# Zhen-Dong/HAWQ

Measured on NVIDIA H100. Metric: images/sec ResNet-50 W8A8 & W4A4 @batch128, 1/2/4/8xH100; % int-TC roofline, higher is better.
Workload: dtype int8

## Files before the change

hawq_b200/csrc/api.cu:

```cuda
#include <cmath>
#include <cstdarg>
#include <cstdio>
#include <cstring>

#include <cstdlib>

#include "conv_igemm.cuh"
#include "elementwise.cuh"
#include "stem.cuh"

using namespace hawq;

struct hawq_handle {
  int device;
  int sm_count;
  int32_t* status;
};

static thread_local char g_err[512] = "";
static long long g_kernel_count[8] = {0, 0, 0, 0, 0, 0, 0, 0};

static int fail(int code, const char* fmt, ...) {
  va_list ap;
  va_start(ap, fmt);
  vsnprintf(g_err, sizeof(g_err), fmt, ap);
  va_end(ap);
  return code;
}

#define CUDA_TRY(expr)                                                                         \
  do {                                                                                         \
    cudaError_t _e = (expr);                                                                   \
    if (_e != cudaSuccess) return fail(HAWQ_ERR_CUDA, "%s: %s", #expr, cudaGetErrorString(_e)); \
  } while (0)

static int launch_check(const char* what) {
  cudaError_t e = cudaGetLastError();
  if (e != cudaSuccess) return fail(HAWQ_ERR_CUDA, "%s launch: %s", what, cudaGetErrorString(e));
  return HAWQ_OK;
}

static int grid_for(long long work_items, int sm_count) {
  long long blocks = (work_items + 255) / 256;
  const long long cap = (long long)sm_count * 16;
  if (blocks > cap) blocks = cap;
  if (blocks < 1) blocks = 1;
  return (int)blocks;
}

template <int BN, bool A4, int FAM, bool DUAL>
static int set_conv_attr1() {
  CUDA_TRY(cudaFuncSetAttribute(conv_igemm_kernel<BN, A4, FAM, DUAL>, cudaFuncAttributeMaxDynamicSharedMemorySize,
                                ConvSmem<BN, A4, DUAL>::TOTAL));
  CUDA_TRY(cudaFuncSetAttribute(conv_igemm_kernel<BN, A4, FAM, DUAL>, cudaFuncAttributePreferredSharedMemoryCarveout,
                                cudaSharedmemCarveoutMaxShared));
  return HAWQ_OK;
}
template <int BN, bool A4>
static int set_conv_attr() {
  int rc;
  if ((rc = set_conv_attr1<BN, A4, FAM_REQUANT, false>()) || (rc = set_conv_attr1<BN, A4, FAM_RESIDUAL, false>()) ||
      (rc = set_conv_attr1<BN, A4, FAM_STORE, false>()))
    return rc;
  return HAWQ_OK;
}

static dim3 conv_grid(long long M, int Cout, int BN) { return dim3((unsigned)((M + CONV_BM - 1) / CONV_BM * (Cout / BN)), 1, 1); }

template <int BN, bool A4>
static void launch_conv(const ConvParams& p, cudaStream_t s) {
  const int smem = ConvSmem<BN, A4, false>::TOTAL;
  const dim3 grid = conv_grid(p.M, p.Cout, BN);
  if (p.mode == HAWQ_EPI_REQUANT) conv_igemm_kernel<BN, A4, FAM_REQUANT, false><<<grid, CONV_THREADS, smem, s>>>(p);
  else if (p.mode == HAWQ_EPI_RESIDUAL) conv_igemm_kernel<BN, A4, FAM_RESIDUAL, false><<<grid, CONV_THREADS, smem, s>>>(p);
  else conv_igemm_kernel<BN, A4, FAM_STORE, false><<<grid, CONV_THREADS, smem, s>>>(p);
}
template <bool A4>
static void launch_conv_dual(const ConvParams& p, cudaStream_t s) {
  conv_igemm_kernel<64, A4, FAM_RESIDUAL, true><<<conv_grid(p.M, p.Cout, 64), CONV_THREADS, ConvSmem<64, A4, true>::TOTAL, s>>>(p);
}

extern "C" {

int hawq_abi_version(void) { return HAWQ_ABI_VERSION; }
const char* hawq_last_error(void) { return g_err; }

int hawq_create(int device, hawq_handle** out) {
  if (!out) return fail(HAWQ_ERR_BAD_ARG, "hawq_create: out is null");
  CUDA_TRY(cudaSetDevice(device));
  cudaDeviceProp prop;
  CUDA_TRY(cudaGetDeviceProperties(&prop, device));
  if (prop.major != 9 || prop.minor != 0)
    return fail(HAWQ_ERR_UNSUPPORTED, "hawq_create: device sm_%d%d is not Hopper sm_90 (the library is built for sm_90a)", prop.major, prop.minor);
  hawq_handle* h = new hawq_handle();
  h->device = device;
  h->sm_count = prop.multiProcessorCount;
  h->status = nullptr;
  CUDA_TRY(cudaMalloc(&h->status, sizeof(int32_t)));
  CUDA_TRY(cudaMemset(h->status, 0, sizeof(int32_t)));
  int rc;
  CUDA_TRY(cudaFuncSetAttribute(linear_dp4a_kernel, cudaFuncAttributeMaxDynamicSharedMemorySize, linear_smem_bytes(LIN_MAX_K)));
  if ((rc = set_conv_attr<128, false>()) || (rc = set_conv_attr<64, false>()) || (rc = set_conv_attr<128, true>()) ||
      (rc = set_conv_attr<64, true>()) || (rc = set_conv_attr1<64, false, FAM_RESIDUAL, true>()) ||
      (rc = set_conv_attr1<64, true, FAM_RESIDUAL, true>()))
    return rc;
  *out = h;
  return HAWQ_OK;
}

int hawq_destroy(hawq_handle* h) {
  if (!h) return HAWQ_OK;
  cudaFree(h->status);
  delete h;
  return HAWQ_OK;
}

int hawq_sm_count(const hawq_handle* h) { return h ? h->sm_count : 0; }

int hawq_reset_status(hawq_handle* h, void* stream) {
  if (!h) return fail(HAWQ_ERR_BAD_ARG, "null handle");
  CUDA_TRY(cudaMemsetAsync(h->status, 0, sizeof(int32_t), (cudaStream_t)stream));
  return HAWQ_OK;
}

int hawq_get_status(hawq_handle* h, void* stream, int32_t* host_flags) {
  if (!h || !host_flags) return fail(HAWQ_ERR_BAD_ARG, "null argument");
  CUDA_TRY(cudaMemcpyAsync(host_flags, h->status, sizeof(int32_t), cudaMemcpyDeviceToHost, (cudaStream_t)stream));
  CUDA_TRY(cudaStreamSynchronize((cudaStream_t)stream));
  return HAWQ_OK;
}

int hawq_copy_status(hawq_handle* h, int32_t* dst, void* stream) {
  if (!h || !dst) return fail(HAWQ_ERR_BAD_ARG, "null argument");
  CUDA_TRY(cudaMemcpyAsync(dst, h->status, sizeof(int32_t), cudaMemcpyDeviceToDevice, (cudaStream_t)stream));
  return HAWQ_OK;
}

static void set_bias_window(ConvParams& p, int a_bits) {
  long long bound = (long long)p.K * (a_bits == 4 ? 15 * 128 : 128 * 128);
  if (bound > 2147483648ll) bound = 2147483648ll;
  p.bias_lo = (int)(bound - 2147483648ll);
  p.bias_hi = (int)(2147483647ll - bound);
}

static int check_me(uint32_t m, int e, const char* what) {
  if (e < 1 || e > 62 || m > 0x80000000u) return fail(HAWQ_ERR_BAD_ARG, "%s: dyadic pair out of range (m=%u e=%d)", what, m, e);
  return HAWQ_OK;
}

int hawq_conv2d(hawq_handle* h, const hawq_conv_desc* d, const hawq_epilogue_desc* ep, const void* x, const int8_t* w,
                const hawq_chan* chan, const void* res, const hawq_chan* res_chan, const float* fscale, void* out,
                void* out_low, void* stream) {
  if (!h || !d || !ep || !x || !w || !chan) return fail(HAWQ_ERR_BAD_ARG, "hawq_conv2d: null argument");
  if (d->N < 1 || d->H < 1 || d->W < 1 || d->kh < 1 || d->kw < 1 || d->stride < 1 || d->pad < 0)
    return fail(HAWQ_ERR_BAD_ARG, "hawq_conv2d: bad geometry");
  if (d->a_bits != 8 && d->a_bits != 4) return fail(HAWQ_ERR_UNSUPPORTED, "hawq_conv2d: a_bits must be 4 or 8");
  if (d->Cin % 64 != 0 || d->Cout % 64 != 0)
    return fail(HAWQ_ERR_UNSUPPORTED, "hawq_conv2d: Cin (%d) and Cout (%d) must be multiples of 64", d->Cin, d->Cout);
  const int Ho = (d->H + 2 * d->pad - d->kh) / d->stride + 1;
  const int Wo = (d->W + 2 * d->pad - d->kw) / d->stride + 1;
  if (Ho < 1 || Wo < 1) return fail(HAWQ_ERR_BAD_ARG, "hawq_conv2d: empty output");
  const long long M = (long long)d->N * Ho * Wo;
  if (M > 0x7fffff00ll || (long long)d->N * d->H * d->W > 0x7fffff00ll) return fail(HAWQ_ERR_UNSUPPORTED, "hawq_conv2d: too many pixels");

  ConvParams p;
  memset(&p, 0, sizeof(p));
  p.x = (const uint8_t*)x; p.w = w; p.chan = chan; p.res = res; p.res_chan = res_chan; p.fscale = fscale;
  p.out = out; p.out_low = out_low; p.status = h->status;
  p.N = d->N; p.H = d->H; p.W = d->W; p.Cin = d->Cin; p.Cout = d->Cout; p.KH = d->kh; p.KW = d->kw;
  p.stride = d->stride; p.pad = d->pad; p.Ho = Ho; p.Wo = Wo; p.M = (int)M; p.K = d->kh * d->kw * d->Cin;
  p.cin_chunks = d->Cin / 64;
  p.x_pix_bytes = d->Cin * d->a_bits / 8;
  p.mode = ep->mode; p.relu = ep->relu; p.out_bits = ep->out_bits; p.lo = ep->clamp_lo; p.hi = ep->clamp_hi;
  p.res_kind = ep->res_kind; p.res_bits = ep->res_bits; p.res_m = ep->res_m; p.res_e = ep->res_e;
  p.y_bits = ep->y_bits; p.low_bits = ep->low_bits; p.low_m = ep->low_m; p.low_e = ep->low_e;
  p.low_lo = ep->low_lo; p.low_hi = ep->low_hi; p.cout_store = ep->cout_store;
  set_bias_window(p, d->a_bits);
  p.check_ovf = ep->mode == HAWQ_EPI_RESIDUAL && (ep->flags & (HAWQ_EP_RATIOS_LE_ONE | HAWQ_EP_RATIOS_LE_2P20)) != 0;
  if (ep->mode == HAWQ_EPI_RESIDUAL) {
    const bool low_over_one = ep->low_bits != 0 && !dyadic_is_fast(ep->low_m, ep->low_e);
    p.scalar_over_one = (ep->res_kind == 0 && !dyadic_is_fast(ep->res_m, ep->res_e)) || low_over_one;
    p.scalar_unchecked = (ep->res_kind == 0 && !dyadic_is_wide(ep->res_m, ep->res_e)) || low_over_one;
  }

  switch (ep->mode) {
    case HAWQ_EPI_REQUANT:
      if (!out) return fail(HAWQ_ERR_BAD_ARG, "hawq_conv2d: REQUANT needs out");
      if (ep->out_bits != 4 && ep->out_bits != 8 && ep->out_bits != 16 && ep->out_bits != 32)
        return fail(HAWQ_ERR_BAD_ARG, "hawq_conv2d: out_bits must be 4/8/16/32");
      if (ep->clamp_lo > ep->clamp_hi) return fail(HAWQ_ERR_BAD_ARG, "hawq_conv2d: empty clamp range");
      break;
    case HAWQ_EPI_RESIDUAL:
      if (!res) return fail(HAWQ_ERR_BAD_ARG, "hawq_conv2d: RESIDUAL needs res");
      if (ep->res_kind == 1) {
        if (!res_chan) return fail(HAWQ_ERR_BAD_ARG, "hawq_conv2d: res_kind 1 needs res_chan");
      } else if (ep->res_kind == 0) {
        if (ep->res_bits != 16 && ep->res_bits != 32) return fail(HAWQ_ERR_BAD_ARG, "hawq_conv2d: res_bits must be 16/32");
        int rc = check_me(ep->res_m, ep->res_e, "hawq_conv2d residual");
        if (rc) return rc;
      } else return fail(HAWQ_ERR_BAD_ARG, "hawq_conv2d: res_kind must be 0/1");
      if (ep->y_bits != 0 && ep->y_bits != 16 && ep->y_bits != 32) return fail(HAWQ_ERR_BAD_ARG, "hawq_conv2d: y_bits must be 0/16/32");
      if (ep->y_bits == 16 && !ep->relu) return fail(HAWQ_ERR_BAD_ARG, "hawq_conv2d: uint16 residual stream requires relu");
      if (ep->y_bits && !out) return fail(HAWQ_ERR_BAD_ARG, "hawq_conv2d: y_bits set but out is null");
      if (ep->low_bits != 0 && ep->low_bits != 4 && ep->low_bits != 8) return fail(HAWQ_ERR_BAD_ARG, "hawq_conv2d: low_bits must be 0/4/8");
      if (ep->low_bits) {
        if (!out_low) return fail(HAWQ_ERR_BAD_ARG, "hawq_conv2d: low_bits set but out_low is null");
        int rc = check_me(ep->low_m, ep->low_e, "hawq_conv2d low-bit copy");
        if (rc) return rc;
      }
      if (!ep->y_bits && !ep->low_bits) return fail(HAWQ_ERR_BAD_ARG, "hawq_conv2d: RESIDUAL with no output");
      break;
    case HAWQ_EPI_RAW_I32:
      if (!out) return fail(HAWQ_ERR_BAD_ARG, "hawq_conv2d: RAW_I32 needs out");
      break;
    case HAWQ_EPI_DEQUANT_F32:
      if (!out || !fscale) return fail(HAWQ_ERR_BAD_ARG, "hawq_conv2d: DEQUANT_F32 needs out and fscale");
      if (ep->cout_store < 1 || ep->cout_store > d->Cout) return fail(HAWQ_ERR_BAD_ARG, "hawq_conv2d: bad cout_store");
      break;
    default:
      return fail(HAWQ_ERR_BAD_ARG, "hawq_conv2d: unknown epilogue mode %d", ep->mode);
  }

  const bool bn128 = (d->Cout % 128 == 0);
  if ((M + CONV_BM - 1) / CONV_BM * (d->Cout / (bn128 ? 128 : 64)) > 0x7fffffffll)
    return fail(HAWQ_ERR_UNSUPPORTED, "hawq_conv2d: more than 2^31 - 1 output tiles");
  ++g_kernel_count[0];
  cudaStream_t s = (cudaStream_t)stream;
  if (d->a_bits == 8) {
    if (bn128) launch_conv<128, false>(p, s);
    else launch_conv<64, false>(p, s);
  } else {
    if (bn128) launch_conv<128, true>(p, s);
    else launch_conv<64, true>(p, s);
  }
  return launch_check("conv_igemm");
}

int hawq_conv2d_dual(hawq_handle* h, const hawq_conv_desc* d, const hawq_epilogue_desc* ep, const void* x, const int8_t* w,
                     const hawq_chan* chan, const hawq_conv_desc* d2, const void* x2, const int8_t* w2, const hawq_chan* chan2,
                     void* out, void* out_low, void* stream) {
  if (!h || !d || !ep || !x || !w || !chan || !d2 || !x2 || !w2 || !chan2 || !out) return fail(HAWQ_ERR_BAD_ARG, "hawq_conv2d_dual: null argument");
  if (d->kh != 1 || d->kw != 1 || d->stride != 1 || d->pad != 0 || d2->kh != 1 || d2->kw != 1 || d2->pad != 0 || d2->stride < 1)
    return fail(HAWQ_ERR_UNSUPPORTED, "hawq_conv2d_dual: both convolutions must be 1x1 without padding (main stride 1)");
  if (d->N < 1 || d->H < 1 || d->W < 1 || d2->H < 1 || d2->W < 1) return fail(HAWQ_ERR_BAD_ARG, "hawq_conv2d_dual: bad geometry");
  if ((d->a_bits != 8 && d->a_bits != 4) || d2->a_bits != d->a_bits) return fail(HAWQ_ERR_UNSUPPORTED, "hawq_conv2d_dual: a_bits must be equal and 4 or 8");
  if (d->Cin % 64 || d2->Cin % 64 || d->Cout % 64 || d2->Cout != d->Cout) return fail(HAWQ_ERR_UNSUPPORTED, "hawq_conv2d_dual: channel counts must be multiples of 64 and Cout equal");
  if (d2->N != d->N || (d2->H - 1) / d2->stride + 1 != d->H || (d2->W - 1) / d2->stride + 1 != d->W)
    return fail(HAWQ_ERR_BAD_ARG, "hawq_conv2d_dual: the two convolutions have different output grids");
  if (d->w_layout != 1 || d2->w_layout != 1) return fail(HAWQ_ERR_UNSUPPORTED, "hawq_conv2d_dual: weights must carry the re-tiled copy (w_layout 1)");
  if (ep->mode != HAWQ_EPI_RESIDUAL || !ep->relu || ep->y_bits != 16) return fail(HAWQ_ERR_UNSUPPORTED, "hawq_conv2d_dual: RESIDUAL + relu + uint16 stream only");
  if (ep->low_bits != 0 && ep->low_bits != 4 && ep->low_bits != 8) return fail(HAWQ_ERR_BAD_ARG, "hawq_conv2d_dual: low_bits must be 0/4/8");
  if (ep->low_bits) {
    if (!out_low) return fail(HAWQ_ERR_BAD_ARG, "hawq_conv2d_dual: low_bits set but out_low is null");
    int rc = check_me(ep->low_m, ep->low_e, "hawq_conv2d_dual low-bit copy");
    if (rc) return rc;
    if (!dyadic_is_fast(ep->low_m, ep->low_e)) return fail(HAWQ_ERR_UNSUPPORTED, "hawq_conv2d_dual: low-bit ratio outside the fast range");
  }
  const bool ratios_one = (ep->flags & HAWQ_EP_RATIOS_LE_ONE) != 0;
  const bool ratios_wide = !ratios_one && (ep->flags & HAWQ_EP_RATIOS_LE_2P20) != 0;
  if (!ratios_one && !ratios_wide) return fail(HAWQ_ERR_UNSUPPORTED, "hawq_conv2d_dual: needs a ratio-range promise (flags)");
  const long long M = (long long)d->N * d->H * d->W;
  if (M > 0x7fffff00ll || (long long)d2->N * d2->H * d2->W > 0x7fffff00ll) return fail(HAWQ_ERR_UNSUPPORTED, "hawq_conv2d_dual: too many pixels");
  if ((M + CONV_BM - 1) / CONV_BM * (d->Cout / 64) > 0x7fffffffll)
    return fail(HAWQ_ERR_UNSUPPORTED, "hawq_conv2d_dual: more than 2^31 - 1 output tiles");

  ++g_kernel_count[4];
  ConvParams p;
  memset(&p, 0, sizeof(p));
  p.x = (const uint8_t*)x; p.w = w; p.chan = chan; p.res_chan = chan2; p.out = out; p.out_low = out_low; p.status = h->status;
  p.N = d->N; p.H = d->H; p.W = d->W; p.Cin = d->Cin; p.Cout = d->Cout; p.KH = 1; p.KW = 1; p.stride = 1; p.pad = 0;
  p.Ho = d->H; p.Wo = d->W; p.M = (int)M; p.K = d->Cin; p.cin_chunks = d->Cin / 64; p.x_pix_bytes = d->Cin * d->a_bits / 8;
  p.mode = HAWQ_EPI_RESIDUAL; p.relu = 1; p.res_kind = 1; p.res_bits = 32; p.y_bits = 16; p.low_bits = ep->low_bits; p.low_m = ep->low_m;
  p.low_e = ep->low_e; p.low_lo = ep->low_lo; p.low_hi = ep->low_hi;
  p.check_ovf = 1;
  set_bias_window(p, d->a_bits);
  p.x2 = (const uint8_t*)x2; p.w2 = w2; p.H2 = d2->H; p.W2 = d2->W; p.stride2 = d2->stride; p.cin_chunks2 = d2->Cin / 64;
  p.x2_pix_bytes = d2->Cin * d2->a_bits / 8;

  cudaStream_t s = (cudaStream_t)stream;
  if (d->a_bits == 8) launch_conv_dual<false>(p, s);
  else launch_conv_dual<true>(p, s);
  return launch_check("conv_dual");
}

int hawq_conv2d_i8(hawq_handle* h, const hawq_conv_desc* d, const hawq_epilogue_desc* ep, const void* x,
                   const int8_t* w, const hawq_chan* chan, const void* res, const hawq_chan* res_chan,
                   const float* fscale, void* out, void* out_low, void* stream) {
  if (d && d->a_bits != 8) return fail(HAWQ_ERR_BAD_ARG, "hawq_conv2d_i8: a_bits must be 8");
  return hawq_conv2d(h, d, ep, x, w, chan, res, res_chan, fscale, out, out_low, stream);
}

int hawq_conv2d_i4(hawq_handle* h, const hawq_conv_desc* d, const hawq_epilogue_desc* ep, const void* x,
                   const int8_t* w, const hawq_chan* chan, const void* res, const hawq_chan* res_chan,
                   const float* fscale, void* out, void* out_low, void* stream) {
  if (d && d->a_bits != 4) return fail(HAWQ_ERR_BAD_ARG, "hawq_conv2d_i4: a_bits must be 4");
  return hawq_conv2d(h, d, ep, x, w, chan, res, res_chan, fscale, out, out_low, stream);
}

int hawq_linear_i8(hawq_handle* h, int32_t N, int32_t K, int32_t Cout, int32_t Cout_pad, const int8_t* x,
                   const int8_t* w, const hawq_chan* chan, const float* fscale, float* out, void* stream) {
  if (Cout < 1 || Cout > Cout_pad) return fail(HAWQ_ERR_BAD_ARG, "hawq_linear_i8: bad Cout/Cout_pad");
  if (!h || !x || !w || !chan || !fscale || !out || N < 1 || K < 1) return fail(HAWQ_ERR_BAD_ARG, "hawq_linear_i8: null argument or empty shape");
  static const bool dp4a_enabled = [] { const char* e = getenv("HAWQ_B200_LINEAR_DP4A"); return !(e && e[0] == '0'); }();
  if (dp4a_enabled && K % LIN_SLAB == 0 && K <= LIN_MAX_K && Cout_pad % LIN_CH == 0 && N <= 65535 * LIN_ROWS) {
    const dim3 grid((unsigned)(Cout_pad / LIN_CH), (unsigned)((N + LIN_ROWS - 1) / LIN_ROWS), 1);
    linear_dp4a_kernel<<<grid, 256, linear_smem_bytes(K), (cudaStream_t)stream>>>(x, w, chan, fscale, out, N, K, Cout);
    return launch_check("linear_dp4a");
  }
  hawq_conv_desc d;
  memset(&d, 0, sizeof(d));
  d.N = N; d.H = 1; d.W = 1; d.Cin = K; d.Cout = Cout_pad; d.kh = 1; d.kw = 1; d.stride = 1; d.pad = 0; d.a_bits = 8;
  hawq_epilogue_desc ep;
  memset(&ep, 0, sizeof(ep));
  ep.mode = HAWQ_EPI_DEQUANT_F32;
  ep.cout_store = Cout;
  return hawq_conv2d(h, &d, &ep, x, w, chan, nullptr, nullptr, fscale, out, nullptr, stream);
}

int hawq_stem_conv_i8(hawq_handle* h, int32_t N, int32_t H, int32_t W, const int8_t* x, const int8_t* w,
                      const hawq_chan* chan, int32_t clamp_lo, int32_t clamp_hi, int16_t* out, void* stream) {
  if (!h || !x || !w || !chan || !out) return fail(HAWQ_ERR_BAD_ARG, "hawq_stem_conv_i8: null argument");
  if (N < 1 || H < 7 || W < 7) return fail(HAWQ_ERR_BAD_ARG, "hawq_stem_conv_i8: bad geometry");
  if (clamp_lo < -32768 || clamp_hi > 32767 || clamp_lo > clamp_hi) return fail(HAWQ_ERR_BAD_ARG, "hawq_stem_conv_i8: clamp must fit int16");
  if (N > 65535) return fail(HAWQ_ERR_UNSUPPORTED, "hawq_stem_conv_i8: N > 65535");
  const int Ho = (H + 6 - 7) / 2 + 1, Wo = (W + 6 - 7) / 2 + 1;
  const dim3 grid((Wo + STEM_TW - 1) / STEM_TW, (Ho + STEM_TH - 1) / STEM_TH, N);
  const long long tiles = (long long)N * grid.x * grid.y;
  const int ctas = (int)(tiles < 4LL * h->sm_count ? tiles : 4LL * h->sm_count);
  stem_conv_kernel<<<ctas, 256, 0, (cudaStream_t)stream>>>(x, (const uint32_t*)w, chan, N, H, W, Ho, Wo, clamp_lo, clamp_hi, out);
  return launch_check("stem_conv");
}

int hawq_stem_pool_i8(hawq_handle* h, int32_t N, int32_t H, int32_t W, const int8_t* x, const int8_t* w256, const hawq_chan* chan,
                      int32_t clamp_lo, int32_t clamp_hi, int32_t y_bits, void* y, int32_t low_bits, uint32_t low_m, int32_t low_e,
                      int32_t low_lo, int32_t low_hi, void* out_low, void* stream) {
  if (!h || !x || !w256 || !chan || !y) return fail(HAWQ_ERR_BAD_ARG, "hawq_stem_pool_i8: null argument");
  if (N < 1 || H < 7 || W < 7) return fail(HAWQ_ERR_BAD_ARG, "hawq_stem_pool_i8: bad geometry");
  if (clamp_lo < -32768 || clamp_hi > 32767 || clamp_lo > clamp_hi) return fail(HAWQ_ERR_BAD_ARG, "hawq_stem_pool_i8: clamp must fit int16");
  if ((y_bits != 16 && y_bits != 32) || (low_bits != 0 && low_bits != 4 && low_bits != 8) || (low_bits && !out_low))
    return fail(HAWQ_ERR_BAD_ARG, "hawq_stem_pool_i8: bad output description");
  if (low_bits) { int rc = check_me(low_m, low_e, "hawq_stem_pool_i8"); if (rc) return rc; }
  if (W % 16 != 0 || W > 256 || (low_bits && !dyadic_is_fast(low_m, low_e)))
    return fail(HAWQ_ERR_UNSUPPORTED, "hawq_stem_pool_i8: shape / ratio outside the fused kernel (use hawq_stem_conv_i8 + hawq_maxpool_requant)");
  if (N > 65535) return fail(HAWQ_ERR_UNSUPPORTED, "hawq_stem_pool_i8: N > 65535");
  const int Ho = (H + 6 - 7) / 2 + 1, Wo = (W + 6 - 7) / 2 + 1;
  const int Po = (Ho + 2 - 3) / 2 + 1, Qo = (Wo + 2 - 3) / 2 + 1;
  const long long tiles = (long long)N * ((Po + STEMP_PH - 1) / STEMP_PH) * ((Qo + STEMP_PW - 1) / STEMP_PW);
  const int ctas = (int)(tiles < 4LL * h->sm_count ? tiles : 4LL * h->sm_count);
  ++g_kernel_count[6];
  stem_pool_kernel<<<ctas, 256, 0, (cudaStream_t)stream>>>(x, (const uint32_t*)w256, chan, N, H, W, Ho, Wo, Po, Qo, clamp_lo, clamp_hi, y_bits, y,
                                                          low_bits, low_m, low_e, low_lo, low_hi, out_low);
  return launch_check("stem_pool");
}

int hawq_maxpool_requant(hawq_handle* h, int32_t N, int32_t H, int32_t W, int32_t C, const int16_t* x, int32_t y_bits,
                         void* y, int32_t low_bits, uint32_t low_m, int32_t low_e, int32_t low_lo, int32_t low_hi,
                         void* out_low, void* stream) {
  if (!h || !x) return fail(HAWQ_ERR_BAD_ARG, "hawq_maxpool_requant: null argument");
  if (C % 8 != 0) return fail(HAWQ_ERR_UNSUPPORTED, "hawq_maxpool_requant: C %% 8 != 0");
  if ((y_bits != 0 && y_bits != 16 && y_bits != 32) || (y_bits && !y)) return fail(HAWQ_ERR_BAD_ARG, "hawq_maxpool_requant: bad y");
  if ((low_bits != 0 && low_bits != 4 && low_bits != 8) || (low_bits && !out_low)) return fail(HAWQ_ERR_BAD_ARG, "hawq_maxpool_requant: bad low");
  if (low_bits) { int rc = check_me(low_m, low_e, "hawq_maxpool_requant"); if (rc) return rc; }
  const int Ho = (H + 2 - 3) / 2 + 1, Wo = (W + 2 - 3) / 2 + 1;
  const long long total = (long long)N * Ho * Wo * (C / 8);
  maxpool_requant_kernel<<<grid_for(total, h->sm_count), 256, 0, (cudaStream_t)stream>>>(
      x, N, H, W, C, Ho, Wo, y_bits, y, low_bits, low_m, low_e, low_lo, low_hi, out_low);
  return launch_check("maxpool_requant");
}

int hawq_avgpool_requant(hawq_handle* h, int32_t N, int32_t HW, int32_t C, int32_t x_bits, const void* x, uint32_t m,
                         int32_t e, int32_t lo, int32_t hi, int8_t* out, void* stream) {
  if (!h || !x || !out) return fail(HAWQ_ERR_BAD_ARG, "hawq_avgpool_requant: null argument");
  if (x_bits != 16 && x_bits != 32) return fail(HAWQ_ERR_BAD_ARG, "hawq_avgpool_requant: x_bits must be 16/32");
  if (lo < -128 || hi > 127) return fail(HAWQ_ERR_BAD_ARG, "hawq_avgpool_requant: clamp must fit int8");
  int rc = check_me(m, e, "hawq_avgpool_requant");
  if (rc) return rc;
  avgpool_requant_kernel<<<grid_for((long long)N * C, h->sm_count), 256, 0, (cudaStream_t)stream>>>(x, N, HW, C, x_bits, m, e, lo, hi, out);
  return launch_check("avgpool_requant");
}

int hawq_quantize_input_f32(hawq_handle* h, int32_t N, int32_t C, int32_t H, int32_t W, const float* x, float scale,
                            int32_t lo, int32_t hi, int8_t* out, void* stream) {
  if (!h || !x || !out) return fail(HAWQ_ERR_BAD_ARG, "hawq_quantize_input_f32: null argument");
  if (!(scale > 0.f)) return fail(HAWQ_ERR_BAD_ARG, "hawq_quantize_input_f32: scale must be > 0");
  if (lo < -128 || hi > 127) return fail(HAWQ_ERR_BAD_ARG, "hawq_quantize_input_f32: clamp must fit int8");
  const float inv = 1.0f / scale;
  quantize_input_kernel<<<grid_for((long long)N * H * W, h->sm_count), 256, 0, (cudaStream_t)stream>>>(x, N, C, H, W, inv, lo, hi, out);
  return launch_check("quantize_input");
}

int hawq_quantize_input_u8(hawq_handle* h, int32_t N, int32_t H, int32_t W, const uint8_t* x, const float* mean3,
                           const float* std3, float scale, int32_t lo, int32_t hi, int8_t* out, void* stream) {
  if (!h || !x || !out || !mean3 || !std3) return fail(HAWQ_ERR_BAD_ARG, "hawq_quantize_input_u8: null argument");
  if (N < 1 || H < 1 || W < 1) return fail(HAWQ_ERR_BAD_ARG, "hawq_quantize_input_u8: empty shape");
  if (!(scale > 0.f)) return fail(HAWQ_ERR_BAD_ARG, "hawq_quantize_input_u8: scale must be > 0");
  if (lo < -128 || hi > 127 || lo > hi) return fail(HAWQ_ERR_BAD_ARG, "hawq_quantize_input_u8: clamp must fit int8");
  for (int c = 0; c < 3; ++c)
    if (!(std3[c] > 0.f)) return fail(HAWQ_ERR_BAD_ARG, "hawq_quantize_input_u8: std must be > 0");
  const float inv = 1.0f / scale;
  const long long n_bytes = (long long)N * H * W * 3;
  quantize_input_u8_kernel<<<grid_for(n_bytes / 4 + 1, h->sm_count), 256, 0, (cudaStream_t)stream>>>(
      x, n_bytes, 3, mean3[0], mean3[1], mean3[2], std3[0], std3[1], std3[2], inv, lo, hi, out);
  return launch_check("quantize_input_u8");
}

int hawq_requant(hawq_handle* h, int64_t rows, int32_t C, int32_t x_bits, const void* x, const hawq_chan* chan,
                 int32_t chan_stride, int32_t relu, int32_t out_bits, int32_t lo, int32_t hi, void* out, void* stream) {
  if (!h || !x || !chan || !out) return fail(HAWQ_ERR_BAD_ARG, "hawq_requant: null argument");
  if (C % 8 != 0) return fail(HAWQ_ERR_UNSUPPORTED, "hawq_requant: C %% 8 != 0");
  if (x_bits != 16 && x_bits != 32) return fail(HAWQ_ERR_BAD_ARG, "hawq_requant: x_bits must be 16/32");
  if (out_bits != 4 && out_bits != 8 && out_bits != 16 && out_bits != 32) return fail(HAWQ_ERR_BAD_ARG, "hawq_requant: out_bits must be 4/8/16/32");
  if (chan_stride != 0 && chan_stride != 1) return fail(HAWQ_ERR_BAD_ARG, "hawq_requant: chan_stride must be 0/1");
  requant_kernel<<<grid_for(rows * (C / 8), h->sm_count), 256, 0, (cudaStream_t)stream>>>(x, rows, C, x_bits, chan, chan_stride, relu, out_bits, lo, hi, out);
  return launch_check("requant");
}

int hawq_add_requant(hawq_handle* h, int64_t rows, int32_t C, const int32_t* acc, const hawq_chan* chan,
                     const hawq_epilogue_desc* ep, const void* res, const hawq_chan* res_chan, void* y, void* out_low,
                     void* stream) {
  if (!h || !acc || !chan || !ep || !res) return fail(HAWQ_ERR_BAD_ARG, "hawq_add_requant: null argument");
  if (C % 8 != 0) return fail(HAWQ_ERR_UNSUPPORTED, "hawq_add_requant: C %% 8 != 0");
  if (ep->res_kind == 1 && !res_chan) return fail(HAWQ_ERR_BAD_ARG, "hawq_add_requant: res_kind 1 needs res_chan");
  if (ep->res_kind == 0) { int rc = check_me(ep->res_m, ep->res_e, "hawq_add_requant"); if (rc) return rc; }
  if (ep->y_bits == 16 && !ep->relu) return fail(HAWQ_ERR_BAD_ARG, "hawq_add_requant: uint16 residual stream requires relu");
  if ((ep->y_bits && !y) || (ep->low_bits && !out_low)) return fail(HAWQ_ERR_BAD_ARG, "hawq_add_requant: missing output");
  AddRequantParams p;
  p.acc = acc; p.chan = chan; p.res = res; p.res_chan = res_chan; p.y = y; p.out_low = out_low; p.status = h->status;
  p.rows = rows; p.C = C; p.relu = ep->relu; p.res_kind = ep->res_kind; p.res_bits = ep->res_bits; p.res_m = ep->res_m;
  p.res_e = ep->res_e; p.y_bits = ep->y_bits; p.low_bits = ep->low_bits; p.low_m = ep->low_m; p.low_e = ep->low_e;
  p.low_lo = ep->low_lo; p.low_hi = ep->low_hi;
  add_requant_kernel<<<grid_for(rows * (C / 8), h->sm_count), 256, 0, (cudaStream_t)stream>>>(p);
  return launch_check("add_requant");
}

int hawq_dequant_f32(hawq_handle* h, int32_t N, int32_t H, int32_t W, int32_t C, int32_t x_bits, int32_t x_signed,
                     const void* x, float scale, float* out_nchw, void* stream) {
  if (!h || !x || !out_nchw) return fail(HAWQ_ERR_BAD_ARG, "hawq_dequant_f32: null argument");
  if (x_bits != 4 && x_bits != 8 && x_bits != 16 && x_bits != 32) return fail(HAWQ_ERR_BAD_ARG, "hawq_dequant_f32: bad x_bits");
  if (x_bits == 4 && C % 8 != 0) return fail(HAWQ_ERR_UNSUPPORTED, "hawq_dequant_f32: packed input needs C %% 8 == 0");
  dequant_f32_kernel<<<grid_for((long long)N * H * W * C, h->sm_count), 256, 0, (cudaStream_t)stream>>>(x, N, H, W, C, x_bits, x_signed, scale, out_nchw);
  return launch_check("dequant_f32");
}

int hawq_pack_i4(hawq_handle* h, int64_t n_values, const uint8_t* in, uint8_t* out, void* stream) {
  if (!h || !in || !out || n_values % 8 != 0) return fail(HAWQ_ERR_BAD_ARG, "hawq_pack_i4: bad argument");
  pack_i4_kernel<<<grid_for(n_values / 8, h->sm_count), 256, 0, (cudaStream_t)stream>>>(in, n_values / 8, out);
  return launch_check("pack_i4");
}

int hawq_unpack_i4(hawq_handle* h, int64_t n_values, const uint8_t* in, uint8_t* out, void* stream) {
  if (!h || !in || !out || n_values % 8 != 0) return fail(HAWQ_ERR_BAD_ARG, "hawq_unpack_i4: bad argument");
  unpack_i4_kernel<<<grid_for(n_values / 8, h->sm_count), 256, 0, (cudaStream_t)stream>>>(in, n_values / 8, out);
  return launch_check("unpack_i4");
}

int hawq_dyadic(double ratio, uint32_t* m, int32_t* e) {
  if (!m || !e || !(ratio > 0.0) || !std::isfinite(ratio)) return fail(HAWQ_ERR_BAD_ARG, "hawq_dyadic: ratio must be positive and finite");
  int ex;
  const double mant = std::frexp(ratio, &ex);
  const double scaled = mant * 2147483648.0;
  const double r = std::floor(scaled + 0.5);
  const int ee = 31 - ex;
  if (ee < 1) return fail(HAWQ_ERR_UNSUPPORTED, "hawq_dyadic: ratio %g too large (e = %d < 1)", ratio, ee);
  if (ee > 62) { *m = 0; *e = 1; return HAWQ_OK; }
  *m = (uint32_t)r;
  *e = ee;
  return HAWQ_OK;
}

int64_t hawq_rhe_requant_host(int32_t v, uint32_t m, int32_t e) { return (int64_t)rhe_requant(v, m, e); }

int hawq_permute_weights_for_i4(int8_t* host_w, int64_t rows_times_taps, int32_t Cin) {
  if (!host_w || Cin % 32 != 0) return fail(HAWQ_ERR_BAD_ARG, "hawq_permute_weights_for_i4: Cin %% 32 != 0");
  int8_t tmp[32];
  for (int64_t r = 0; r < rows_times_taps; ++r) {
    for (int blk = 0; blk < Cin / 32; ++blk) {
      int8_t* p = host_w + r * Cin + blk * 32;
      for (int t = 0; t < 4; ++t)
        for (int j = 0; j < 4; ++j) {
          tmp[4 * t + j] = p[8 * t + j];
          tmp[16 + 4 * t + j] = p[8 * t + 4 + j];
        }
      memcpy(p, tmp, 32);
    }
  }
  return HAWQ_OK;
}

int64_t hawq_workspace_bytes(const hawq_conv_desc*, const hawq_epilogue_desc*) { return 0; }

int hawq_retile_weights(hawq_handle* h, const int8_t* w_ohwi, int32_t Cout, int64_t K, int8_t* out, void* stream) {
  if (!h || !w_ohwi || !out) return fail(HAWQ_ERR_BAD_ARG, "hawq_retile_weights: null argument");
  if (Cout % 64 != 0 || K % 64 != 0) return fail(HAWQ_ERR_UNSUPPORTED, "hawq_retile_weights: Cout and K must be multiples of 64");
  const int bn = (Cout % 128 == 0) ? 128 : 64;
  const long long chunks = (long long)Cout * K / 16;
  retile_weights_kernel<<<grid_for(chunks, h->sm_count), 256, 0, (cudaStream_t)stream>>>(w_ohwi, Cout, (int)K, bn, out);
  return launch_check("retile_weights");
}


int64_t hawq_debug_kernel_count(int32_t family) { return (family >= 0 && family < 8) ? g_kernel_count[family] : -1; }

}
```

hawq_b200/csrc/conv_igemm.cuh:

```cuda
#pragma once
#include <type_traits>

#include "common.cuh"
#include "wgmma.cuh"

namespace hawq {

struct ConvParams {
  const uint8_t* x;
  const int8_t* w;
  const hawq_chan* chan;
  const void* res;
  const hawq_chan* res_chan;
  const float* fscale;
  void* out;
  void* out_low;
  int32_t* status;
  int N, H, W, Cin, Cout, KH, KW, stride, pad, Ho, Wo, M, K;
  int cin_chunks;
  int x_pix_bytes;
  int mode, relu, out_bits, lo, hi;
  int res_kind, res_bits;
  uint32_t res_m;
  int res_e;
  int y_bits, low_bits;
  uint32_t low_m;
  int low_e, low_lo, low_hi;
  int cout_store;
  int scalar_over_one;
  int scalar_unchecked;
  int check_ovf;
  int bias_lo, bias_hi;
  const uint8_t* x2;
  const int8_t* w2;
  int H2, W2, stride2, cin_chunks2, x2_pix_bytes;
};

constexpr int CONV_BM = 128;
constexpr int CONV_STAGES = 4;
constexpr int CONV_THREADS = 256;

template <int BN, bool A4, bool DUAL>
struct ConvSmem {
  static constexpr int A_ROW = A4 ? 32 : 64;
  static constexpr int A_STAGE = CONV_BM * A_ROW;
  static constexpr int B_STAGE = BN * 64;
  static constexpr int PIPE = CONV_STAGES * (A_STAGE + B_STAGE);
  static constexpr int OUT_PITCH = BN + 16;
  static constexpr int OUT_STAGE = CONV_BM * OUT_PITCH;
  static constexpr int RES16 = CONV_BM * (BN * 2 + 16);
  static constexpr int RES32 = CONV_BM * (BN * 4 + 32);
  static constexpr int RES16_OFF = PIPE;
  static constexpr int RES32_OFF = DUAL ? PIPE : OUT_STAGE;
  static constexpr int Y_OFF = OUT_STAGE;
  static constexpr int MAIN = DUAL ? PIPE + RES32 : (PIPE + RES16 > RES32_OFF + RES32 ? PIPE + RES16 : RES32_OFF + RES32);
  static constexpr int CHAN_OFF = MAIN;
  static constexpr int M_OFF = CHAN_OFF + BN * (int)sizeof(hawq_chan);
  static constexpr int M1_OFF = M_OFF + BN * 8;
  static constexpr int RC_OFF = M1_OFF + BN * 8;
  static constexpr int CB_OFF = RC_OFF + BN * (int)sizeof(hawq_chan);
  static constexpr int TOTAL = CB_OFF + BN * 8;
  static_assert(OUT_STAGE <= PIPE && (!DUAL || Y_OFF + RES16 <= PIPE), "the epilogue staging tiles must fit in the freed ring");
  static_assert(2 * (TOTAL + 1024) <= 228 * 1024, "two CTAs per SM must fit in shared memory");
};

template <int ROW_BYTES>
__device__ __forceinline__ int swz(int row, int ch) {
  if constexpr (ROW_BYTES == 64) return row * 64 + ((ch ^ ((row >> 1) & 3)) << 4);
  else return row * 32 + ((ch ^ ((row >> 2) & 1)) << 4);
}

constexpr int FAM_REQUANT = 0, FAM_RESIDUAL = 1, FAM_STORE = 2;

template <bool CLAMPED>
struct RqFp64 {
  bool checked;
  bool ovf = false;
  static constexpr double kMagic = 6755399441055744.0;
  __device__ static double acc_bias(int32_t acc, double cb, int32_t) {
    const double d = __hiloint2double(0x43300000, acc ^ 0x80000000) - cb;
    return CLAMPED ? fmin(fmax(d, -2147483648.0), 2147483647.0) : d;
  }
  __device__ static double of_i32(int32_t v) {
    return __hiloint2double(0x43300000, v ^ 0x80000000) - 4503601774854144.0;
  }
  __device__ static double of_u16(uint32_t u) { return __hiloint2double(0x43300000, (int)u) - 4503599627370496.0; }
  __device__ int32_t term(double d, double M, uint32_t, int32_t, bool count) {
    const double t = __fma_rn(d, M, kMagic);
    if (checked && count) {
      const double q = t - kMagic;
      ovf |= q > 2147483647.0 || q < -2147483648.0;
    }
    return __double2loint(t);
  }
};
struct RqExact {
  bool checked;
  bool ovf = false;
  __device__ static int32_t acc_bias(int32_t acc, double, int32_t bias) { return sat_add(acc, bias); }
  __device__ static int32_t of_i32(int32_t v) { return v; }
  __device__ static int32_t of_u16(uint32_t u) { return (int32_t)u; }
  __device__ int32_t term(int32_t v, double, uint32_t m, int32_t e, bool count) {
    const long long q = rhe_requant64(v, m, e);
    if (checked && count) ovf |= q > 2147483647ll || q < -2147483648ll;
    return sat_i32(q);
  }
};

struct ConvGeom {
  const uint8_t* x;
  const int8_t* w;
  int H, W, stride, pad, KH, KW, cin_chunks, x_pix_bytes, K;
};

template <int BN, bool A4, int FAM, bool DUAL>
__global__ void __launch_bounds__(CONV_THREADS, 2) conv_igemm_kernel(const ConvParams p) {
  using S = ConvSmem<BN, A4, DUAL>;
  constexpr int BM = CONV_BM, STAGES = CONV_STAGES;
  constexpr int A_ROW = S::A_ROW;
  constexpr int A_CH = A_ROW / 16;
  constexpr int A_ROWS_PER_PASS = CONV_THREADS / A_CH;
  constexpr int A_PASSES = BM / A_ROWS_PER_PASS;
  constexpr int B_PASSES = BN / 64;
  constexpr int NT = BN / 8;
  constexpr int NACC = BN / 2;

  extern __shared__ __align__(1024) uint8_t smem[];
  uint8_t* sA = smem;
  uint8_t* sB = smem + STAGES * S::A_STAGE;
  hawq_chan* sChan = reinterpret_cast<hawq_chan*>(smem + S::CHAN_OFF);
  double* sM = reinterpret_cast<double*>(smem + S::M_OFF);
  double* sM1 = reinterpret_cast<double*>(smem + S::M1_OFF);
  hawq_chan* sResChan = reinterpret_cast<hawq_chan*>(smem + S::RC_OFF);
  double* sCb = reinterpret_cast<double*>(smem + S::CB_OFF);

  const int tid = threadIdx.x;
  const int lane = tid & 31, warp = tid >> 5;
  const int wg = warp >> 2;
  const int g = lane >> 2, t = lane & 3;
  const int nblk = p.Cout / BN;
  const int m0 = (int)(blockIdx.x / nblk) * BM;
  const int n0 = (int)(blockIdx.x % nblk) * BN;

  int over_one = p.scalar_over_one;
  int unchecked = p.scalar_unchecked;
  int bias_out = 0;
  if (tid < BN) {
    const hawq_chan c = p.chan[n0 + tid];
    sChan[tid] = c;
    sM[tid] = dyadic_to_double(c.m, c.e);
    sCb[tid] = 4503601774854144.0 - (double)c.bias;
    bias_out = c.bias < p.bias_lo || c.bias > p.bias_hi;
    over_one |= !dyadic_is_fast(c.m, c.e);
    unchecked |= !dyadic_is_wide(c.m, c.e);
    if (FAM == FAM_RESIDUAL && p.res_kind == 1) {
      const hawq_chan rc = p.res_chan[n0 + tid];
      sResChan[tid] = rc;
      sM1[tid] = dyadic_to_double(rc.m, rc.e);
      over_one |= !dyadic_is_fast(rc.m, rc.e);
      unchecked |= !dyadic_is_wide(rc.m, rc.e);
    }
  }
  const bool ratio_over_one = __syncthreads_or(over_one) != 0;
  const bool ratio_unchecked = __syncthreads_or(unchecked) != 0;
  const bool clamped = __syncthreads_or(bias_out) != 0;
  const bool fp64 = !ratio_over_one || (FAM == FAM_RESIDUAL && p.check_ovf && !ratio_unchecked);

  int32_t acc[NACC];

  const int res_es = (FAM == FAM_RESIDUAL) ? ((p.res_kind == 1 || p.res_bits == 32) ? 4 : 2) : 0;
  const int res_pitch = BN * res_es + 8 * res_es;
  uint8_t* sRes = smem + (res_es == 2 ? S::RES16_OFF : S::RES32_OFF);

  auto load_res = [&]() {
    if constexpr (FAM == FAM_RESIDUAL) {
      const int cpr = BN * res_es / 16;
      const uint8_t* gres = reinterpret_cast<const uint8_t*>(p.res);
      for (int id = tid; id < BM * cpr; id += CONV_THREADS) {
        const int row = id / cpr, j = id - row * cpr;
        const bool v = m0 + row < p.M;
        const uint8_t* src = v ? gres + ((size_t)(m0 + row) * p.Cout + n0) * res_es + j * 16 : gres;
        cp_async_16(smem_u32(sRes + row * res_pitch + j * 16), src, v ? 16 : 0);
      }
    }
  };
  const bool prefetch_res = !DUAL && res_es == 2;

  auto gemm = [&](const ConvGeom& gm, bool with_res) {
#pragma unroll
    for (int i = 0; i < NACC; ++i) acc[i] = 0;
    const int a_ch = tid % A_CH;
    int a_hi0[A_PASSES], a_wi0[A_PASSES], a_pix[A_PASSES];
    bool a_ok[A_PASSES];
#pragma unroll
    for (int i = 0; i < A_PASSES; ++i) {
      const int row = tid / A_CH + i * A_ROWS_PER_PASS;
      const int m = m0 + row;
      a_ok[i] = m < p.M;
      const int mm = a_ok[i] ? m : 0;
      const int n = mm / (p.Ho * p.Wo);
      const int r = mm - n * (p.Ho * p.Wo);
      const int ho = r / p.Wo, wo = r - ho * p.Wo;
      a_hi0[i] = ho * gm.stride - gm.pad;
      a_wi0[i] = wo * gm.stride - gm.pad;
      a_pix[i] = n * gm.H * gm.W;
    }
    const int b_ch = tid & 3, b_row = tid >> 2;
    const int KT = gm.KH * gm.KW * gm.cin_chunks;
    int ld_c = 0, ld_kw = 0, ld_kh = 0, ld_kt = 0;

    auto load_tile = [&](int stage) {
      const uint32_t a_base = smem_u32(sA + stage * S::A_STAGE);
#pragma unroll
      for (int i = 0; i < A_PASSES; ++i) {
        const int row = tid / A_CH + i * A_ROWS_PER_PASS;
        const int hi = a_hi0[i] + ld_kh, wi = a_wi0[i] + ld_kw;
        const bool v = a_ok[i] && (unsigned)hi < (unsigned)gm.H && (unsigned)wi < (unsigned)gm.W;
        const uint8_t* src = gm.x;
        if (v) src = gm.x + (size_t)(a_pix[i] + hi * gm.W + wi) * gm.x_pix_bytes + ld_c * A_ROW + a_ch * 16;
        cp_async_16(a_base + swz<A_ROW>(row, a_ch), src, v ? 16 : 0);
      }
      const uint32_t b_base = smem_u32(sB + stage * S::B_STAGE);
#pragma unroll
      for (int i = 0; i < B_PASSES; ++i) {
        const int row = b_row + i * 64;
        const int8_t* src = gm.w + (size_t)(n0 + row) * gm.K + ld_kt * 64 + b_ch * 16;
        cp_async_16(b_base + swz<64>(row, b_ch), src, 16);
      }
      ++ld_kt;
      if (++ld_c == gm.cin_chunks) {
        ld_c = 0;
        if (++ld_kw == gm.KW) { ld_kw = 0; ++ld_kh; }
      }
    };

#pragma unroll
    for (int s = 0; s < STAGES - 1; ++s) {
      if (s < KT) load_tile(s);
      if (s == STAGES - 2 && with_res) load_res();
      cp_async_commit();
    }

    for (int kt = 0; kt < KT; ++kt) {
      cp_async_wait<STAGES - 2>();
      fence_proxy_async_smem();
      __syncthreads();
      if (kt + STAGES - 1 < KT) load_tile((kt + STAGES - 1) % STAGES);
      cp_async_commit();

      const int stage = kt % STAGES;
      const uint32_t a_base = smem_u32(sA + stage * S::A_STAGE);
      const uint32_t b_base = smem_u32(sB + stage * S::B_STAGE);
#pragma unroll
      for (int ks = 0; ks < 2; ++ks) {
        const uint64_t bdesc = wgmma_desc_sw64(b_base + ks * 32);
        if constexpr (!A4) {
          wgmma_fence();
          wgmma_ss<BN>(acc, wgmma_desc_sw64(a_base + wg * 64 * A_ROW + ks * 32), bdesc);
        } else {
          uint32_t r0, r1;
          const int row = warp * 16 + (lane & 7) + ((lane >> 3) & 1) * 8;
          ldmatrix_x2(r0, r1, a_base + swz<32>(row, ks));
          const uint32_t af[4] = {r0 & 0x0F0F0F0Fu, r1 & 0x0F0F0F0Fu, (r0 >> 4) & 0x0F0F0F0Fu, (r1 >> 4) & 0x0F0F0F0Fu};
          wgmma_fence();
          wgmma_rs<BN>(acc, af, bdesc);
        }
      }
      wgmma_commit();
      wgmma_wait_all();
      fence_operands(acc);
    }
    cp_async_wait<0>();
    __syncthreads();
  };

  if constexpr (DUAL) {
    gemm(ConvGeom{p.x2, p.w2, p.H2, p.W2, p.stride2, 0, 1, 1, p.cin_chunks2, p.x2_pix_bytes, p.cin_chunks2 * 64}, false);
#pragma unroll
    for (int ni = 0; ni < NT; ++ni) {
      const int col = ni * 8 + 2 * t;
      const int b0 = sResChan[col].bias, b1 = sResChan[col + 1].bias;
#pragma unroll
      for (int hf = 0; hf < 2; ++hf) {
        const int row = warp * 16 + hf * 8 + g;
        *reinterpret_cast<int2*>(sRes + row * res_pitch + col * 4) =
            make_int2(sat_add(acc[ni * 4 + hf * 2], b0), sat_add(acc[ni * 4 + hf * 2 + 1], b1));
      }
    }
  }
  gemm(ConvGeom{p.x, p.w, p.H, p.W, p.stride, p.pad, p.KH, p.KW, p.cin_chunks, p.x_pix_bytes, p.K}, prefetch_res);

  if (!DUAL && res_es == 4) {
    load_res();
    cp_async_commit();
    cp_async_wait<0>();
    __syncthreads();
  }
  const bool y_staged = DUAL || (res_es != 0 && p.y_bits == res_es * 8);
  const int y_es = p.y_bits / 8;
  const int y_pitch = BN * y_es + 8 * y_es;
  uint8_t* sY = DUAL ? smem + S::Y_OFF : sRes;

  uint8_t* sOut = smem;
  const bool stage_low = (FAM == FAM_REQUANT && p.out_bits <= 8) || (FAM == FAM_RESIDUAL && p.low_bits != 0);
  const int stage_bits = (FAM == FAM_REQUANT) ? p.out_bits : p.low_bits;

  auto put_low = [&](int row, int col, int q0, int q1) {
    *reinterpret_cast<uint16_t*>(sOut + row * S::OUT_PITCH + col) = (uint16_t)__byte_perm(q0, q1, 0x0040);
  };
  auto put_y = [&](int row, int col, bool ok, int y0, int y1, int& ymax) {
    if (p.y_bits == 16 && ok) ymax = max(ymax, max(y0, y1));
    if (!y_staged && !ok) return;
    uint8_t* dst = y_staged ? sY + row * y_pitch + col * y_es
                            : reinterpret_cast<uint8_t*>(p.out) + ((size_t)(m0 + row) * p.Cout + n0 + col) * y_es;
    if (p.y_bits == 16) *reinterpret_cast<uint32_t*>(dst) = (uint32_t)min(y0, 65535) | ((uint32_t)min(y1, 65535) << 16);
    else if (p.y_bits == 32) *reinterpret_cast<int2*>(dst) = make_int2(y0, y1);
  };

  auto epilogue = [&](auto rq, auto low_out) {
    if constexpr (FAM == FAM_REQUANT) {
      const int lo = p.relu ? min(max(p.lo, 0), p.hi) : p.lo;
#pragma unroll
      for (int ni = 0; ni < NT; ++ni) {
        const int col = ni * 8 + 2 * t;
        const int4 c0 = *reinterpret_cast<const int4*>(&sChan[col]);
        const int4 c1 = *reinterpret_cast<const int4*>(&sChan[col + 1]);
        const double2 M = *reinterpret_cast<const double2*>(&sM[col]);
        const double2 Cb = *reinterpret_cast<const double2*>(&sCb[col]);
#pragma unroll
        for (int hf = 0; hf < 2; ++hf) {
          const int row = warp * 16 + hf * 8 + g;
          const int q0 = clampi(rq.term(rq.acc_bias(acc[ni * 4 + hf * 2], Cb.x, c0.x), M.x, c0.y, c0.z, false), lo, p.hi);
          const int q1 = clampi(rq.term(rq.acc_bias(acc[ni * 4 + hf * 2 + 1], Cb.y, c1.x), M.y, c1.y, c1.z, false), lo, p.hi);
          if constexpr (decltype(low_out)::value) {
            put_low(row, col, q0, q1);
          } else if (m0 + row < p.M) {
            uint8_t* dst = reinterpret_cast<uint8_t*>(p.out) + ((size_t)(m0 + row) * p.Cout + n0 + col) * (p.out_bits / 8);
            if (p.out_bits == 16) *reinterpret_cast<uint32_t*>(dst) = (uint32_t)(q0 & 0xFFFF) | ((uint32_t)q1 << 16);
            else *reinterpret_cast<int2*>(dst) = make_int2(q0, q1);
          }
        }
      }
    } else {
      const double res_M = dyadic_to_double(p.res_m, p.res_e), low_M = dyadic_to_double(p.low_m, p.low_e);
      const int relu_floor = p.relu ? 0 : (int)0x80000000;
      int ymax = 0;
#pragma unroll
      for (int ni = 0; ni < NT; ++ni) {
        const int col = ni * 8 + 2 * t;
        const int4 c0 = *reinterpret_cast<const int4*>(&sChan[col]);
        const int4 c1 = *reinterpret_cast<const int4*>(&sChan[col + 1]);
        const double2 M = *reinterpret_cast<const double2*>(&sM[col]);
        const double2 Cb = *reinterpret_cast<const double2*>(&sCb[col]);
        double2 M1 = make_double2(res_M, res_M);
        uint2 m1 = make_uint2(p.res_m, p.res_m);
        int2 e1 = make_int2(p.res_e, p.res_e);
        if (p.res_kind == 1) {
          M1 = *reinterpret_cast<const double2*>(&sM1[col]);
          m1 = make_uint2(sResChan[col].m, sResChan[col + 1].m);
          e1 = make_int2(sResChan[col].e, sResChan[col + 1].e);
        }
#pragma unroll
        for (int hf = 0; hf < 2; ++hf) {
          const int row = warp * 16 + hf * 8 + g;
          const bool ok = m0 + row < p.M;
          const uint8_t* rptr = sRes + row * res_pitch + col * res_es;
          decltype(rq.of_i32(0)) r0, r1;
          if (res_es == 2) {
            const uint32_t pr = *reinterpret_cast<const uint32_t*>(rptr);
            r0 = rq.of_u16(pr & 0xFFFFu);
            r1 = rq.of_u16(pr >> 16);
          } else {
            const int2 pr = *reinterpret_cast<const int2*>(rptr);
            r0 = rq.of_i32(pr.x);
            r1 = rq.of_i32(pr.y);
          }
          const auto v0 = rq.acc_bias(acc[ni * 4 + hf * 2 + 0], Cb.x, c0.x);
          const auto v1 = rq.acc_bias(acc[ni * 4 + hf * 2 + 1], Cb.y, c1.x);
          const int y0 = max(sat_add(rq.term(r0, M1.x, m1.x, e1.x, ok), rq.term(v0, M.x, c0.y, c0.z, ok)), relu_floor);
          const int y1 = max(sat_add(rq.term(r1, M1.y, m1.y, e1.y, ok), rq.term(v1, M.y, c1.y, c1.z, ok)), relu_floor);
          put_y(row, col, ok, y0, y1, ymax);
          if (p.low_bits != 0)
            put_low(row, col, clampi(rq.term(rq.of_i32(y0), low_M, p.low_m, p.low_e, false), p.low_lo, p.low_hi),
                    clampi(rq.term(rq.of_i32(y1), low_M, p.low_m, p.low_e, false), p.low_lo, p.low_hi));
        }
      }
      if (ymax > 65535) atomicOr(p.status, HAWQ_FLAG_RESIDUAL_OVERFLOW);
      if (rq.ovf) atomicOr(p.status, HAWQ_FLAG_REQUANT_OVERFLOW);
    }
  };

  if constexpr (FAM == FAM_STORE) {
#pragma unroll
    for (int ni = 0; ni < NT; ++ni) {
      const int col = ni * 8 + 2 * t;
      const int b0 = sChan[col].bias, b1 = sChan[col + 1].bias;
#pragma unroll
      for (int hf = 0; hf < 2; ++hf) {
        const int m = m0 + warp * 16 + hf * 8 + g;
        if (m >= p.M) continue;
        const int32_t v0 = sat_add(acc[ni * 4 + hf * 2 + 0], b0), v1 = sat_add(acc[ni * 4 + hf * 2 + 1], b1);
        if (p.mode == HAWQ_EPI_RAW_I32) {
          *reinterpret_cast<int2*>(reinterpret_cast<int32_t*>(p.out) + (size_t)m * p.Cout + n0 + col) = make_int2(v0, v1);
        } else {
          float* o = reinterpret_cast<float*>(p.out) + (size_t)m * p.cout_store;
          const int c = n0 + col;
          if (c < p.cout_store) o[c] = __fmul_rn((float)v0, p.fscale[c]);
          if (c + 1 < p.cout_store) o[c + 1] = __fmul_rn((float)v1, p.fscale[c + 1]);
        }
      }
    }
  } else {
    auto run = [&](auto low_out) {
      if (!fp64) epilogue(RqExact{FAM == FAM_RESIDUAL && p.check_ovf}, low_out);
      else if (clamped) epilogue(RqFp64<true>{FAM == FAM_RESIDUAL && ratio_over_one}, low_out);
      else epilogue(RqFp64<false>{FAM == FAM_RESIDUAL && ratio_over_one}, low_out);
    };
    if (FAM == FAM_REQUANT && p.out_bits <= 8) run(std::true_type{});
    else run(std::false_type{});
  }

  if (y_staged || stage_low) __syncthreads();
  if (y_staged) {
    const int cpr = BN * y_es / 16;
    uint8_t* gy = reinterpret_cast<uint8_t*>(p.out);
    for (int id = tid; id < BM * cpr; id += CONV_THREADS) {
      const int row = id / cpr, j = id - row * cpr;
      if (m0 + row < p.M)
        *reinterpret_cast<int4*>(gy + ((size_t)(m0 + row) * p.Cout + n0) * y_es + j * 16) =
            *reinterpret_cast<const int4*>(sY + row * y_pitch + j * 16);
    }
  }
  if (stage_low) {
    uint8_t* gout = reinterpret_cast<uint8_t*>(FAM == FAM_REQUANT ? p.out : p.out_low);
    if (stage_bits == 8) {
      constexpr int CPR = BN / 16;
      for (int id = tid; id < BM * CPR; id += CONV_THREADS) {
        const int row = id / CPR, j = id % CPR;
        if (m0 + row < p.M) {
          const int4 v = *reinterpret_cast<const int4*>(sOut + row * S::OUT_PITCH + j * 16);
          *reinterpret_cast<int4*>(gout + (size_t)(m0 + row) * p.Cout + n0 + j * 16) = v;
        }
      }
    } else {
      constexpr int CPR = BN / 32;
      for (int id = tid; id < BM * CPR; id += CONV_THREADS) {
        const int row = id / CPR, j = id % CPR;
        if (m0 + row < p.M) {
          const uint4 a = *reinterpret_cast<const uint4*>(sOut + row * S::OUT_PITCH + j * 32);
          const uint4 b = *reinterpret_cast<const uint4*>(sOut + row * S::OUT_PITCH + j * 32 + 16);
          uint4 o;
          o.x = pack_nibbles8(a.x, a.y);
          o.y = pack_nibbles8(a.z, a.w);
          o.z = pack_nibbles8(b.x, b.y);
          o.w = pack_nibbles8(b.z, b.w);
          *reinterpret_cast<uint4*>(gout + (((size_t)(m0 + row) * p.Cout + n0 + j * 32) >> 1)) = o;
        }
      }
    }
  }
}

}
```

Baseline: 25280.

## Add persistent tail kernel for 1x1 residual convs with cross-tile pipelining

Adds a persistent conv_tail_kernel for 1x1 stride-1 residual convolutions with 16-bit residual and output, and for the dual (projection shortcut) convolution. A fixed grid of about two CTAs per SM walks row tiles for one channel block. It loads the channel parameters once and streams cp.async loads continuously across tiles, so the next tile's operands and residual prefetch overlap the current tile's epilogue. This is meant to remove per-tile launch, prologue and pipeline-drain costs on the short-K bottleneck tail convolutions. The generic kernel loses its DUAL specialisation, and shared channel and epilogue helpers are factored out.

```diff
diff --git a/hawq_b200/csrc/api.cu b/hawq_b200/csrc/api.cu
--- a/hawq_b200/csrc/api.cu
+++ b/hawq_b200/csrc/api.cu
@@ -6,6 +6,7 @@
 #include <cstdlib>
 
 #include "conv_igemm.cuh"
+#include "conv_tail.cuh"
 #include "elementwise.cuh"
 #include "stem.cuh"
 
@@ -48,19 +49,20 @@
   return (int)blocks;
 }
 
-template <int BN, bool A4, int FAM, bool DUAL>
-static int set_conv_attr1() {
-  CUDA_TRY(cudaFuncSetAttribute(conv_igemm_kernel<BN, A4, FAM, DUAL>, cudaFuncAttributeMaxDynamicSharedMemorySize,
-                                ConvSmem<BN, A4, DUAL>::TOTAL));
-  CUDA_TRY(cudaFuncSetAttribute(conv_igemm_kernel<BN, A4, FAM, DUAL>, cudaFuncAttributePreferredSharedMemoryCarveout,
-                                cudaSharedmemCarveoutMaxShared));
+template <class K>
+static int set_smem_attr(K* kernel, int smem) {
+  CUDA_TRY(cudaFuncSetAttribute(kernel, cudaFuncAttributeMaxDynamicSharedMemorySize, smem));
+  CUDA_TRY(cudaFuncSetAttribute(kernel, cudaFuncAttributePreferredSharedMemoryCarveout, cudaSharedmemCarveoutMaxShared));
   return HAWQ_OK;
 }
 template <int BN, bool A4>
 static int set_conv_attr() {
+  constexpr int smem = ConvSmem<BN, A4>::TOTAL;
   int rc;
-  if ((rc = set_conv_attr1<BN, A4, FAM_REQUANT, false>()) || (rc = set_conv_attr1<BN, A4, FAM_RESIDUAL, false>()) ||
-      (rc = set_conv_attr1<BN, A4, FAM_STORE, false>()))
+  if ((rc = set_smem_attr(conv_igemm_kernel<BN, A4, FAM_REQUANT>, smem)) || (rc = set_smem_attr(conv_igemm_kernel<BN, A4, FAM_RESIDUAL>, smem)) ||
+      (rc = set_smem_attr(conv_igemm_kernel<BN, A4, FAM_STORE>, smem)) ||
+      (rc = set_smem_attr(conv_tail_kernel<A4, false>, TailSmem<A4, false>::TOTAL)) ||
+      (rc = set_smem_attr(conv_tail_kernel<A4, true>, TailSmem<A4, true>::TOTAL)))
     return rc;
   return HAWQ_OK;
 }
@@ -69,15 +71,15 @@
 
 template <int BN, bool A4>
 static void launch_conv(const ConvParams& p, cudaStream_t s) {
-  const int smem = ConvSmem<BN, A4, false>::TOTAL;
+  const int smem = ConvSmem<BN, A4>::TOTAL;
   const dim3 grid = conv_grid(p.M, p.Cout, BN);
-  if (p.mode == HAWQ_EPI_REQUANT) conv_igemm_kernel<BN, A4, FAM_REQUANT, false><<<grid, CONV_THREADS, smem, s>>>(p);
-  else if (p.mode == HAWQ_EPI_RESIDUAL) conv_igemm_kernel<BN, A4, FAM_RESIDUAL, false><<<grid, CONV_THREADS, smem, s>>>(p);
-  else conv_igemm_kernel<BN, A4, FAM_STORE, false><<<grid, CONV_THREADS, smem, s>>>(p);
-}
-template <bool A4>
-static void launch_conv_dual(const ConvParams& p, cudaStream_t s) {
-  conv_igemm_kernel<64, A4, FAM_RESIDUAL, true><<<conv_grid(p.M, p.Cout, 64), CONV_THREADS, ConvSmem<64, A4, true>::TOTAL, s>>>(p);
+  if (p.mode == HAWQ_EPI_REQUANT) conv_igemm_kernel<BN, A4, FAM_REQUANT><<<grid, CONV_THREADS, smem, s>>>(p);
+  else if (p.mode == HAWQ_EPI_RESIDUAL) conv_igemm_kernel<BN, A4, FAM_RESIDUAL><<<grid, CONV_THREADS, smem, s>>>(p);
+  else conv_igemm_kernel<BN, A4, FAM_STORE><<<grid, CONV_THREADS, smem, s>>>(p);
+}
+template <bool A4, bool DUAL>
+static void launch_conv_tail(const ConvParams& p, int sm_count, cudaStream_t s) {
+  conv_tail_kernel<A4, DUAL><<<tail_grid(p.Cout, sm_count), CONV_THREADS, TailSmem<A4, DUAL>::TOTAL, s>>>(p);
 }
 
 extern "C" {
@@ -101,8 +103,7 @@
   int rc;
   CUDA_TRY(cudaFuncSetAttribute(linear_dp4a_kernel, cudaFuncAttributeMaxDynamicSharedMemorySize, linear_smem_bytes(LIN_MAX_K)));
   if ((rc = set_conv_attr<128, false>()) || (rc = set_conv_attr<64, false>()) || (rc = set_conv_attr<128, true>()) ||
-      (rc = set_conv_attr<64, true>()) || (rc = set_conv_attr1<64, false, FAM_RESIDUAL, true>()) ||
-      (rc = set_conv_attr1<64, true, FAM_RESIDUAL, true>()))
+      (rc = set_conv_attr<64, true>()))
     return rc;
   *out = h;
   return HAWQ_OK;
@@ -157,6 +158,7 @@
   if (d->a_bits != 8 && d->a_bits != 4) return fail(HAWQ_ERR_UNSUPPORTED, "hawq_conv2d: a_bits must be 4 or 8");
   if (d->Cin % 64 != 0 || d->Cout % 64 != 0)
     return fail(HAWQ_ERR_UNSUPPORTED, "hawq_conv2d: Cin (%d) and Cout (%d) must be multiples of 64", d->Cin, d->Cout);
+  if (d->Cin < 64 || d->Cout < 64) return fail(HAWQ_ERR_BAD_ARG, "hawq_conv2d: Cin (%d) and Cout (%d) must be at least 64", d->Cin, d->Cout);
   const int Ho = (d->H + 2 * d->pad - d->kh) / d->stride + 1;
   const int Wo = (d->W + 2 * d->pad - d->kw) / d->stride + 1;
   if (Ho < 1 || Wo < 1) return fail(HAWQ_ERR_BAD_ARG, "hawq_conv2d: empty output");
@@ -226,7 +228,12 @@
     return fail(HAWQ_ERR_UNSUPPORTED, "hawq_conv2d: more than 2^31 - 1 output tiles");
   ++g_kernel_count[0];
   cudaStream_t s = (cudaStream_t)stream;
-  if (d->a_bits == 8) {
+  const bool tail = ep->mode == HAWQ_EPI_RESIDUAL && d->kh == 1 && d->kw == 1 && d->stride == 1 && d->pad == 0 && ep->res_kind == 0 &&
+                    ep->res_bits == 16 && ep->y_bits == 16;
+  if (tail) {
+    if (d->a_bits == 8) launch_conv_tail<false, false>(p, h->sm_count, s);
+    else launch_conv_tail<true, false>(p, h->sm_count, s);
+  } else if (d->a_bits == 8) {
     if (bn128) launch_conv<128, false>(p, s);
     else launch_conv<64, false>(p, s);
   } else {
@@ -245,6 +252,7 @@
   if (d->N < 1 || d->H < 1 || d->W < 1 || d2->H < 1 || d2->W < 1) return fail(HAWQ_ERR_BAD_ARG, "hawq_conv2d_dual: bad geometry");
   if ((d->a_bits != 8 && d->a_bits != 4) || d2->a_bits != d->a_bits) return fail(HAWQ_ERR_UNSUPPORTED, "hawq_conv2d_dual: a_bits must be equal and 4 or 8");
   if (d->Cin % 64 || d2->Cin % 64 || d->Cout % 64 || d2->Cout != d->Cout) return fail(HAWQ_ERR_UNSUPPORTED, "hawq_conv2d_dual: channel counts must be multiples of 64 and Cout equal");
+  if (d->Cin < 64 || d2->Cin < 64 || d->Cout < 64) return fail(HAWQ_ERR_BAD_ARG, "hawq_conv2d_dual: Cin and Cout must be at least 64");
   if (d2->N != d->N || (d2->H - 1) / d2->stride + 1 != d->H || (d2->W - 1) / d2->stride + 1 != d->W)
     return fail(HAWQ_ERR_BAD_ARG, "hawq_conv2d_dual: the two convolutions have different output grids");
   if (d->w_layout != 1 || d2->w_layout != 1) return fail(HAWQ_ERR_UNSUPPORTED, "hawq_conv2d_dual: weights must carry the re-tiled copy (w_layout 1)");
@@ -278,8 +286,8 @@
   p.x2_pix_bytes = d2->Cin * d2->a_bits / 8;
 
   cudaStream_t s = (cudaStream_t)stream;
-  if (d->a_bits == 8) launch_conv_dual<false>(p, s);
-  else launch_conv_dual<true>(p, s);
+  if (d->a_bits == 8) launch_conv_tail<false, true>(p, h->sm_count, s);
+  else launch_conv_tail<true, true>(p, h->sm_count, s);
   return launch_check("conv_dual");
 }
 
diff --git a/hawq_b200/csrc/conv_igemm.cuh b/hawq_b200/csrc/conv_igemm.cuh
--- a/hawq_b200/csrc/conv_igemm.cuh
+++ b/hawq_b200/csrc/conv_igemm.cuh
@@ -40,7 +40,25 @@
 constexpr int CONV_STAGES = 4;
 constexpr int CONV_THREADS = 256;
 
-template <int BN, bool A4, bool DUAL>
+template <int BN>
+struct ChanSmem {
+  static constexpr int M_OFF = BN * (int)sizeof(hawq_chan);
+  static constexpr int M1_OFF = M_OFF + BN * 8;
+  static constexpr int RC_OFF = M1_OFF + BN * 8;
+  static constexpr int CB_OFF = RC_OFF + BN * (int)sizeof(hawq_chan);
+  static constexpr int BYTES = CB_OFF + BN * 8;
+  hawq_chan* chan;
+  double* M;
+  double* M1;
+  hawq_chan* rc;
+  double* Cb;
+  __device__ explicit ChanSmem(uint8_t* base)
+      : chan(reinterpret_cast<hawq_chan*>(base)), M(reinterpret_cast<double*>(base + M_OFF)),
+        M1(reinterpret_cast<double*>(base + M1_OFF)), rc(reinterpret_cast<hawq_chan*>(base + RC_OFF)),
+        Cb(reinterpret_cast<double*>(base + CB_OFF)) {}
+};
+
+template <int BN, bool A4>
 struct ConvSmem {
   static constexpr int A_ROW = A4 ? 32 : 64;
   static constexpr int A_STAGE = CONV_BM * A_ROW;
@@ -51,16 +69,11 @@
   static constexpr int RES16 = CONV_BM * (BN * 2 + 16);
   static constexpr int RES32 = CONV_BM * (BN * 4 + 32);
   static constexpr int RES16_OFF = PIPE;
-  static constexpr int RES32_OFF = DUAL ? PIPE : OUT_STAGE;
-  static constexpr int Y_OFF = OUT_STAGE;
-  static constexpr int MAIN = DUAL ? PIPE + RES32 : (PIPE + RES16 > RES32_OFF + RES32 ? PIPE + RES16 : RES32_OFF + RES32);
+  static constexpr int RES32_OFF = OUT_STAGE;
+  static constexpr int MAIN = PIPE + RES16 > RES32_OFF + RES32 ? PIPE + RES16 : RES32_OFF + RES32;
   static constexpr int CHAN_OFF = MAIN;
-  static constexpr int M_OFF = CHAN_OFF + BN * (int)sizeof(hawq_chan);
-  static constexpr int M1_OFF = M_OFF + BN * 8;
-  static constexpr int RC_OFF = M1_OFF + BN * 8;
-  static constexpr int CB_OFF = RC_OFF + BN * (int)sizeof(hawq_chan);
-  static constexpr int TOTAL = CB_OFF + BN * 8;
-  static_assert(OUT_STAGE <= PIPE && (!DUAL || Y_OFF + RES16 <= PIPE), "the epilogue staging tiles must fit in the freed ring");
+  static constexpr int TOTAL = CHAN_OFF + ChanSmem<BN>::BYTES;
+  static_assert(OUT_STAGE <= PIPE, "the low-bit staging tile must fit in the freed ring");
   static_assert(2 * (TOTAL + 1024) <= 228 * 1024, "two CTAs per SM must fit in shared memory");
 };
 
@@ -107,15 +120,107 @@
   }
 };
 
+struct RqPolicy {
+  bool over_one;
+  bool unchecked;
+  bool clamped;
+};
+
+template <int BN, bool RESIDUAL>
+__device__ RqPolicy load_channel_block(const ConvParams& p, int n0, const ChanSmem<BN>& cs) {
+  int over_one = p.scalar_over_one, unchecked = p.scalar_unchecked, bias_out = 0;
+  const int tid = threadIdx.x;
+  if (tid < BN) {
+    const hawq_chan c = p.chan[n0 + tid];
+    cs.chan[tid] = c;
+    cs.M[tid] = dyadic_to_double(c.m, c.e);
+    cs.Cb[tid] = 4503601774854144.0 - (double)c.bias;
+    bias_out = c.bias < p.bias_lo || c.bias > p.bias_hi;
+    over_one |= !dyadic_is_fast(c.m, c.e);
+    unchecked |= !dyadic_is_wide(c.m, c.e);
+    if (RESIDUAL && p.res_kind == 1) {
+      const hawq_chan rc = p.res_chan[n0 + tid];
+      cs.rc[tid] = rc;
+      cs.M1[tid] = dyadic_to_double(rc.m, rc.e);
+      over_one |= !dyadic_is_fast(rc.m, rc.e);
+      unchecked |= !dyadic_is_wide(rc.m, rc.e);
+    }
+  }
+  RqPolicy pol;
+  pol.over_one = __syncthreads_or(over_one) != 0;
+  pol.unchecked = __syncthreads_or(unchecked) != 0;
+  pol.clamped = __syncthreads_or(bias_out) != 0;
+  return pol;
+}
+
+template <bool RESIDUAL, class F>
+__device__ __forceinline__ void with_rq(const RqPolicy& pol, const ConvParams& p, F&& f) {
+  const bool fp64 = !pol.over_one || (RESIDUAL && p.check_ovf && !pol.unchecked);
+  if (!fp64) f(RqExact{RESIDUAL && p.check_ovf != 0});
+  else if (pol.clamped) f(RqFp64<true>{RESIDUAL && pol.over_one});
+  else f(RqFp64<false>{RESIDUAL && pol.over_one});
+}
+
+template <class Rq>
+__device__ __forceinline__ int32_t residual_y(Rq& rq, int32_t res_term, int32_t acc, double cb, const int4& c, double M, bool ok,
+                                              int32_t relu_floor) {
+  return max(sat_add(res_term, rq.term(rq.acc_bias(acc, cb, c.x), M, c.y, c.z, ok)), relu_floor);
+}
+template <class Rq>
+__device__ __forceinline__ int32_t residual_low(Rq& rq, int32_t y, double low_M, const ConvParams& p) {
+  return clampi(rq.term(rq.of_i32(y), low_M, p.low_m, p.low_e, false), p.low_lo, p.low_hi);
+}
+__device__ __forceinline__ uint32_t stream16_pair(int32_t y0, int32_t y1, bool ok, int& ymax) {
+  if (ok) ymax = max(ymax, max(y0, y1));
+  return (uint32_t)min(y0, 65535) | ((uint32_t)min(y1, 65535) << 16);
+}
+__device__ __forceinline__ void residual_flags(const ConvParams& p, int ymax, bool ovf) {
+  if (ymax > 65535) atomicOr(p.status, HAWQ_FLAG_RESIDUAL_OVERFLOW);
+  if (ovf) atomicOr(p.status, HAWQ_FLAG_REQUANT_OVERFLOW);
+}
+__device__ __forceinline__ void stage_low_pair(uint8_t* s, int pitch, int row, int col, int q0, int q1) {
+  *reinterpret_cast<uint16_t*>(s + row * pitch + col) = (uint16_t)__byte_perm(q0, q1, 0x0040);
+}
+
+__device__ __forceinline__ void copy_out_rows(const uint8_t* s, int s_pitch, uint8_t* g, size_t g_pitch, int row_bytes, int m0, int M) {
+  const int cpr = row_bytes / 16;
+  for (int id = threadIdx.x; id < CONV_BM * cpr; id += blockDim.x) {
+    const int row = id / cpr, j = id - row * cpr;
+    if (m0 + row < M)
+      *reinterpret_cast<int4*>(g + (size_t)(m0 + row) * g_pitch + j * 16) = *reinterpret_cast<const int4*>(s + row * s_pitch + j * 16);
+  }
+}
+template <int BN>
+__device__ __forceinline__ void copy_out_low(const uint8_t* s, int pitch, uint8_t* gout, int bits, int m0, int n0, int M, int Cout) {
+  if (bits == 8) {
+    copy_out_rows(s, pitch, gout + n0, (size_t)Cout, BN, m0, M);
+  } else {
+    constexpr int CPR = BN / 32;
+    for (int id = threadIdx.x; id < CONV_BM * CPR; id += blockDim.x) {
+      const int row = id / CPR, j = id % CPR;
+      if (m0 + row < M) {
+        const uint4 a = *reinterpret_cast<const uint4*>(s + row * pitch + j * 32);
+        const uint4 b = *reinterpret_cast<const uint4*>(s + row * pitch + j * 32 + 16);
+        uint4 o;
+        o.x = pack_nibbles8(a.x, a.y);
+        o.y = pack_nibbles8(a.z, a.w);
+        o.z = pack_nibbles8(b.x, b.y);
+        o.w = pack_nibbles8(b.z, b.w);
+        *reinterpret_cast<uint4*>(gout + (((size_t)(m0 + row) * Cout + n0 + j * 32) >> 1)) = o;
+      }
+    }
+  }
+}
+
 struct ConvGeom {
   const uint8_t* x;
   const int8_t* w;
   int H, W, stride, pad, KH, KW, cin_chunks, x_pix_bytes, K;
 };
 
-template <int BN, bool A4, int FAM, bool DUAL>
+template <int BN, bool A4, int FAM>
 __global__ void __launch_bounds__(CONV_THREADS, 2) conv_igemm_kernel(const ConvParams p) {
-  using S = ConvSmem<BN, A4, DUAL>;
+  using S = ConvSmem<BN, A4>;
   constexpr int BM = CONV_BM, STAGES = CONV_STAGES;
   constexpr int A_ROW = S::A_ROW;
   constexpr int A_CH = A_ROW / 16;
@@ -128,11 +233,12 @@
   extern __shared__ __align__(1024) uint8_t smem[];
   uint8_t* sA = smem;
   uint8_t* sB = smem + STAGES * S::A_STAGE;
-  hawq_chan* sChan = reinterpret_cast<hawq_chan*>(smem + S::CHAN_OFF);
-  double* sM = reinterpret_cast<double*>(smem + S::M_OFF);
-  double* sM1 = reinterpret_cast<double*>(smem + S::M1_OFF);
-  hawq_chan* sResChan = reinterpret_cast<hawq_chan*>(smem + S::RC_OFF);
-  double* sCb = reinterpret_cast<double*>(smem + S::CB_OFF);
+  const ChanSmem<BN> cs(smem + S::CHAN_OFF);
+  const hawq_chan* sChan = cs.chan;
+  const double* sM = cs.M;
+  const double* sM1 = cs.M1;
+  const hawq_chan* sResChan = cs.rc;
+  const double* sCb = cs.Cb;
 
   const int tid = threadIdx.x;
   const int lane = tid & 31, warp = tid >> 5;
@@ -142,29 +248,7 @@
   const int m0 = (int)(blockIdx.x / nblk) * BM;
   const int n0 = (int)(blockIdx.x % nblk) * BN;
 
-  int over_one = p.scalar_over_one;
-  int unchecked = p.scalar_unchecked;
-  int bias_out = 0;
-  if (tid < BN) {
-    const hawq_chan c = p.chan[n0 + tid];
-    sChan[tid] = c;
-    sM[tid] = dyadic_to_double(c.m, c.e);
-    sCb[tid] = 4503601774854144.0 - (double)c.bias;
-    bias_out = c.bias < p.bias_lo || c.bias > p.bias_hi;
-    over_one |= !dyadic_is_fast(c.m, c.e);
-    unchecked |= !dyadic_is_wide(c.m, c.e);
-    if (FAM == FAM_RESIDUAL && p.res_kind == 1) {
-      const hawq_chan rc = p.res_chan[n0 + tid];
-      sResChan[tid] = rc;
-      sM1[tid] = dyadic_to_double(rc.m, rc.e);
-      over_one |= !dyadic_is_fast(rc.m, rc.e);
-      unchecked |= !dyadic_is_wide(rc.m, rc.e);
-    }
-  }
-  const bool ratio_over_one = __syncthreads_or(over_one) != 0;
-  const bool ratio_unchecked = __syncthreads_or(unchecked) != 0;
-  const bool clamped = __syncthreads_or(bias_out) != 0;
-  const bool fp64 = !ratio_over_one || (FAM == FAM_RESIDUAL && p.check_ovf && !ratio_unchecked);
+  const RqPolicy pol = load_channel_block<BN, FAM == FAM_RESIDUAL>(p, n0, cs);
 
   int32_t acc[NACC];
 
@@ -184,7 +268,7 @@
       }
     }
   };
-  const bool prefetch_res = !DUAL && res_es == 2;
+  const bool prefetch_res = res_es == 2;
 
   auto gemm = [&](const ConvGeom& gm, bool with_res) {
 #pragma unroll
@@ -274,46 +358,30 @@
     __syncthreads();
   };
 
-  if constexpr (DUAL) {
-    gemm(ConvGeom{p.x2, p.w2, p.H2, p.W2, p.stride2, 0, 1, 1, p.cin_chunks2, p.x2_pix_bytes, p.cin_chunks2 * 64}, false);
-#pragma unroll
-    for (int ni = 0; ni < NT; ++ni) {
-      const int col = ni * 8 + 2 * t;
-      const int b0 = sResChan[col].bias, b1 = sResChan[col + 1].bias;
-#pragma unroll
-      for (int hf = 0; hf < 2; ++hf) {
-        const int row = warp * 16 + hf * 8 + g;
-        *reinterpret_cast<int2*>(sRes + row * res_pitch + col * 4) =
-            make_int2(sat_add(acc[ni * 4 + hf * 2], b0), sat_add(acc[ni * 4 + hf * 2 + 1], b1));
-      }
-    }
-  }
   gemm(ConvGeom{p.x, p.w, p.H, p.W, p.stride, p.pad, p.KH, p.KW, p.cin_chunks, p.x_pix_bytes, p.K}, prefetch_res);
 
-  if (!DUAL && res_es == 4) {
+  if (res_es == 4) {
     load_res();
     cp_async_commit();
     cp_async_wait<0>();
     __syncthreads();
   }
-  const bool y_staged = DUAL || (res_es != 0 && p.y_bits == res_es * 8);
+  const bool y_staged = res_es != 0 && p.y_bits == res_es * 8;
   const int y_es = p.y_bits / 8;
   const int y_pitch = BN * y_es + 8 * y_es;
-  uint8_t* sY = DUAL ? smem + S::Y_OFF : sRes;
+  uint8_t* sY = sRes;
 
   uint8_t* sOut = smem;
   const bool stage_low = (FAM == FAM_REQUANT && p.out_bits <= 8) || (FAM == FAM_RESIDUAL && p.low_bits != 0);
   const int stage_bits = (FAM == FAM_REQUANT) ? p.out_bits : p.low_bits;
 
-  auto put_low = [&](int row, int col, int q0, int q1) {
-    *reinterpret_cast<uint16_t*>(sOut + row * S::OUT_PITCH + col) = (uint16_t)__byte_perm(q0, q1, 0x0040);
-  };
+  auto put_low = [&](int row, int col, int q0, int q1) { stage_low_pair(sOut, S::OUT_PITCH, row, col, q0, q1); };
   auto put_y = [&](int row, int col, bool ok, int y0, int y1, int& ymax) {
-    if (p.y_bits == 16 && ok) ymax = max(ymax, max(y0, y1));
+    const uint32_t y16 = p.y_bits == 16 ? stream16_pair(y0, y1, ok, ymax) : 0u;
     if (!y_staged && !ok) return;
     uint8_t* dst = y_staged ? sY + row * y_pitch + col * y_es
                             : reinterpret_cast<uint8_t*>(p.out) + ((size_t)(m0 + row) * p.Cout + n0 + col) * y_es;
-    if (p.y_bits == 16) *reinterpret_cast<uint32_t*>(dst) = (uint32_t)min(y0, 65535) | ((uint32_t)min(y1, 65535) << 16);
+    if (p.y_bits == 16) *reinterpret_cast<uint32_t*>(dst) = y16;
     else if (p.y_bits == 32) *reinterpret_cast<int2*>(dst) = make_int2(y0, y1);
   };
 
@@ -375,18 +443,13 @@
             r0 = rq.of_i32(pr.x);
             r1 = rq.of_i32(pr.y);
           }
-          const auto v0 = rq.acc_bias(acc[ni * 4 + hf * 2 + 0], Cb.x, c0.x);
-          const auto v1 = rq.acc_bias(acc[ni * 4 + hf * 2 + 1], Cb.y, c1.x);
-          const int y0 = max(sat_add(rq.term(r0, M1.x, m1.x, e1.x, ok), rq.term(v0, M.x, c0.y, c0.z, ok)), relu_floor);
-          const int y1 = max(sat_add(rq.term(r1, M1.y, m1.y, e1.y, ok), rq.term(v1, M.y, c1.y, c1.z, ok)), relu_floor);
+          const int y0 = residual_y(rq, rq.term(r0, M1.x, m1.x, e1.x, ok), acc[ni * 4 + hf * 2 + 0], Cb.x, c0, M.x, ok, relu_floor);
+          const int y1 = residual_y(rq, rq.term(r1, M1.y, m1.y, e1.y, ok), acc[ni * 4 + hf * 2 + 1], Cb.y, c1, M.y, ok, relu_floor);
           put_y(row, col, ok, y0, y1, ymax);
-          if (p.low_bits != 0)
-            put_low(row, col, clampi(rq.term(rq.of_i32(y0), low_M, p.low_m, p.low_e, false), p.low_lo, p.low_hi),
-                    clampi(rq.term(rq.of_i32(y1), low_M, p.low_m, p.low_e, false), p.low_lo, p.low_hi));
+          if (p.low_bits != 0) put_low(row, col, residual_low(rq, y0, low_M, p), residual_low(rq, y1, low_M, p));
         }
       }
-      if (ymax > 65535) atomicOr(p.status, HAWQ_FLAG_RESIDUAL_OVERFLOW);
-      if (rq.ovf) atomicOr(p.status, HAWQ_FLAG_REQUANT_OVERFLOW);
+      residual_flags(p, ymax, rq.ovf);
     }
   };
 
@@ -411,54 +474,16 @@
       }
     }
   } else {
-    auto run = [&](auto low_out) {
-      if (!fp64) epilogue(RqExact{FAM == FAM_RESIDUAL && p.check_ovf}, low_out);
-      else if (clamped) epilogue(RqFp64<true>{FAM == FAM_RESIDUAL && ratio_over_one}, low_out);
-      else epilogue(RqFp64<false>{FAM == FAM_RESIDUAL && ratio_over_one}, low_out);
-    };
+    auto run = [&](auto low_out) { with_rq<FAM == FAM_RESIDUAL>(pol, p, [&](auto rq) { epilogue(rq, low_out); }); };
     if (FAM == FAM_REQUANT && p.out_bits <= 8) run(std::true_type{});
     else run(std::false_type{});
   }
 
   if (y_staged || stage_low) __syncthreads();
-  if (y_staged) {
-    const int cpr = BN * y_es / 16;
-    uint8_t* gy = reinterpret_cast<uint8_t*>(p.out);
-    for (int id = tid; id < BM * cpr; id += CONV_THREADS) {
-      const int row = id / cpr, j = id - row * cpr;
-      if (m0 + row < p.M)
-        *reinterpret_cast<int4*>(gy + ((size_t)(m0 + row) * p.Cout + n0) * y_es + j * 16) =
-            *reinterpret_cast<const int4*>(sY + row * y_pitch + j * 16);
-    }
-  }
-  if (stage_low) {
-    uint8_t* gout = reinterpret_cast<uint8_t*>(FAM == FAM_REQUANT ? p.out : p.out_low);
-    if (stage_bits == 8) {
-      constexpr int CPR = BN / 16;
-      for (int id = tid; id < BM * CPR; id += CONV_THREADS) {
-        const int row = id / CPR, j = id % CPR;
-        if (m0 + row < p.M) {
-          const int4 v = *reinterpret_cast<const int4*>(sOut + row * S::OUT_PITCH + j * 16);
-          *reinterpret_cast<int4*>(gout + (size_t)(m0 + row) * p.Cout + n0 + j * 16) = v;
-        }
-      }
-    } else {
-      constexpr int CPR = BN / 32;
-      for (int id = tid; id < BM * CPR; id += CONV_THREADS) {
-        const int row = id / CPR, j = id % CPR;
-        if (m0 + row < p.M) {
-          const uint4 a = *reinterpret_cast<const uint4*>(sOut + row * S::OUT_PITCH + j * 32);
-          const uint4 b = *reinterpret_cast<const uint4*>(sOut + row * S::OUT_PITCH + j * 32 + 16);
-          uint4 o;
-          o.x = pack_nibbles8(a.x, a.y);
-          o.y = pack_nibbles8(a.z, a.w);
-          o.z = pack_nibbles8(b.x, b.y);
-          o.w = pack_nibbles8(b.z, b.w);
-          *reinterpret_cast<uint4*>(gout + (((size_t)(m0 + row) * p.Cout + n0 + j * 32) >> 1)) = o;
-        }
-      }
-    }
-  }
-}
-
-}
+  if (y_staged)
+    copy_out_rows(sY, y_pitch, reinterpret_cast<uint8_t*>(p.out) + (size_t)n0 * y_es, (size_t)p.Cout * y_es, BN * y_es, m0, p.M);
+  if (stage_low)
+    copy_out_low<BN>(sOut, S::OUT_PITCH, reinterpret_cast<uint8_t*>(FAM == FAM_REQUANT ? p.out : p.out_low), stage_bits, m0, n0, p.M, p.Cout);
+}
+
+}
diff --git a/hawq_b200/csrc/conv_tail.cuh b/hawq_b200/csrc/conv_tail.cuh
--- /dev/null
+++ b/hawq_b200/csrc/conv_tail.cuh
@@ -0,0 +1,224 @@
+#pragma once
+#include "conv_igemm.cuh"
+
+namespace hawq {
+
+constexpr int TAIL_BN = 64;
+
+template <bool A4, bool DUAL>
+struct TailSmem {
+  static constexpr int BN = TAIL_BN;
+  static constexpr int A_ROW = A4 ? 32 : 64;
+  static constexpr int A_STAGE = CONV_BM * A_ROW;
+  static constexpr int B_STAGE = BN * 64;
+  static constexpr int PIPE = CONV_STAGES * (A_STAGE + B_STAGE);
+  static constexpr int Y_PITCH = BN * 2 + 16;
+  static constexpr int Y_SLOT = CONV_BM * Y_PITCH;
+  static constexpr int I_OFF = PIPE;
+  static constexpr int Y_OFF = I_OFF + (DUAL ? BN / 4 * CONV_THREADS * 8 : 0);
+  static constexpr int Y_SLOTS = DUAL ? 1 : 2;
+  static constexpr int OUT_PITCH = BN + 16;
+  static constexpr int OUT_OFF = Y_OFF + Y_SLOTS * Y_SLOT;
+  static constexpr int CHAN_OFF = OUT_OFF + CONV_BM * OUT_PITCH;
+  static constexpr int TOTAL = CHAN_OFF + ChanSmem<BN>::BYTES;
+  static_assert(A_STAGE % 512 == 0 && B_STAGE % 512 == 0, "wgmma tiles must stay 512-B aligned");
+  static_assert(Y_OFF % 16 == 0 && Y_SLOT % 16 == 0 && OUT_OFF % 16 == 0 && CHAN_OFF % 16 == 0, "16-byte copies need aligned tiles");
+  static_assert(2 * (TOTAL + 1024) <= 228 * 1024, "two CTAs per SM must fit in shared memory");
+};
+
+inline int tail_grid(int Cout, int sm_count) {
+  const int nblk = Cout / TAIL_BN;
+  const int per = 2 * sm_count / nblk;
+  return (per > 1 ? per : 1) * nblk;
+}
+
+template <bool A4, bool DUAL>
+__global__ void __launch_bounds__(CONV_THREADS, 2) conv_tail_kernel(const ConvParams p) {
+  using S = TailSmem<A4, DUAL>;
+  constexpr int BN = TAIL_BN, BM = CONV_BM, STAGES = CONV_STAGES;
+  constexpr int A_ROW = S::A_ROW;
+  constexpr int A_CH = A_ROW / 16;
+  constexpr int A_ROWS_PER_PASS = CONV_THREADS / A_CH;
+  constexpr int A_PASSES = BM / A_ROWS_PER_PASS;
+  constexpr int NT = BN / 8;
+  constexpr int NACC = BN / 2;
+
+  extern __shared__ __align__(1024) uint8_t smem[];
+  uint8_t* sA = smem;
+  uint8_t* sB = smem + STAGES * S::A_STAGE;
+  uint8_t* sOut = smem + S::OUT_OFF;
+  const ChanSmem<BN> cs(smem + S::CHAN_OFF);
+
+  const int tid = threadIdx.x;
+  const int lane = tid & 31, warp = tid >> 5;
+  const int wg = warp >> 2;
+  const int g = lane >> 2, t = lane & 3;
+
+  const int nblk = p.Cout / BN;
+  const int n0 = (int)(blockIdx.x % nblk) * BN;
+  const int rt0 = (int)(blockIdx.x / nblk), rstep = (int)(gridDim.x / nblk);
+  const int nrt = (p.M + BM - 1) / BM;
+  if (rt0 >= nrt) return;
+  const int T = (nrt - rt0 + rstep - 1) / rstep;
+
+  const RqPolicy pol = load_channel_block<BN, true>(p, n0, cs);
+
+  const int KT = p.cin_chunks;
+  const int KT2 = DUAL ? p.cin_chunks2 : 0;
+  const int KTT = KT + KT2;
+  const int D = DUAL ? STAGES - 1 : min(STAGES - 1, KT);
+
+  int ld_t = 0, ld_k = 0, ld_s = 0;
+  int ld_pix2[A_PASSES];
+  const int a_ch = tid % A_CH;
+  const int b_ch = tid & 3, b_row = tid >> 2;
+  auto issue = [&]() {
+    if (ld_t < T) {
+      const int lm0 = (rt0 + ld_t * rstep) * BM;
+      const bool ident = DUAL && ld_k < KT2;
+      const int kc = ident ? ld_k : ld_k - KT2;
+      const uint8_t* xb = ident ? p.x2 : p.x;
+      const int pix_bytes = ident ? p.x2_pix_bytes : p.x_pix_bytes;
+      const uint32_t a_base = smem_u32(sA + ld_s * S::A_STAGE);
+#pragma unroll
+      for (int i = 0; i < A_PASSES; ++i) {
+        const int row = tid / A_CH + i * A_ROWS_PER_PASS;
+        const int m = lm0 + row;
+        const bool v = m < p.M;
+        if (DUAL && ld_k == 0 && v) {
+          const int n = m / (p.Ho * p.Wo);
+          const int r = m - n * (p.Ho * p.Wo);
+          const int ho = r / p.Wo, wo = r - ho * p.Wo;
+          ld_pix2[i] = (n * p.H2 + ho * p.stride2) * p.W2 + wo * p.stride2;
+        }
+        const uint8_t* src = xb;
+        if (v) src = xb + (size_t)(ident ? ld_pix2[i] : m) * pix_bytes + kc * A_ROW + a_ch * 16;
+        cp_async_16(a_base + swz<A_ROW>(row, a_ch), src, v ? 16 : 0);
+      }
+      const int8_t* wb = ident ? p.w2 : p.w;
+      const int wk = (ident ? KT2 : KT) * 64;
+      cp_async_16(smem_u32(sB + ld_s * S::B_STAGE) + swz<64>(b_row, b_ch), wb + (size_t)(n0 + b_row) * wk + kc * 64 + b_ch * 16, 16);
+      if (!DUAL && ld_k == 0) {
+        uint8_t* sr = smem + S::Y_OFF + (ld_t & 1) * S::Y_SLOT;
+        const uint8_t* gres = reinterpret_cast<const uint8_t*>(p.res);
+        constexpr int CPR = BN * 2 / 16;
+        for (int id = tid; id < BM * CPR; id += CONV_THREADS) {
+          const int row = id / CPR, j = id - row * CPR;
+          const bool v = lm0 + row < p.M;
+          const uint8_t* src = v ? gres + ((size_t)(lm0 + row) * p.Cout + n0) * 2 + j * 16 : gres;
+          cp_async_16(smem_u32(sr + row * S::Y_PITCH + j * 16), src, v ? 16 : 0);
+        }
+      }
+      if (++ld_k == KTT) { ld_k = 0; ++ld_t; }
+      if (++ld_s == STAGES) ld_s = 0;
+    }
+    cp_async_commit();
+  };
+
+  int32_t acc[NACC];
+  int cs_s = 0;
+  auto consume = [&]() {
+    if (D == 1) cp_async_wait<0>();
+    else if (D == 2) cp_async_wait<1>();
+    else cp_async_wait<2>();
+    fence_proxy_async_smem();
+    __syncthreads();
+    issue();
+    const uint32_t a_base = smem_u32(sA + cs_s * S::A_STAGE);
+    const uint32_t b_base = smem_u32(sB + cs_s * S::B_STAGE);
+    if (++cs_s == STAGES) cs_s = 0;
+#pragma unroll
+    for (int ks = 0; ks < 2; ++ks) {
+      const uint64_t bdesc = wgmma_desc_sw64(b_base + ks * 32);
+      if constexpr (!A4) {
+        wgmma_fence();
+        wgmma_ss<BN>(acc, wgmma_desc_sw64(a_base + wg * 64 * A_ROW + ks * 32), bdesc);
+      } else {
+        uint32_t r0, r1;
+        const int row = warp * 16 + (lane & 7) + ((lane >> 3) & 1) * 8;
+        ldmatrix_x2(r0, r1, a_base + swz<32>(row, ks));
+        const uint32_t af[4] = {r0 & 0x0F0F0F0Fu, r1 & 0x0F0F0F0Fu, (r0 >> 4) & 0x0F0F0F0Fu, (r1 >> 4) & 0x0F0F0F0Fu};
+        wgmma_fence();
+        wgmma_rs<BN>(acc, af, bdesc);
+      }
+    }
+    wgmma_commit();
+    wgmma_wait_all();
+    fence_operands(acc);
+  };
+
+  for (int s = 0; s < D; ++s) issue();
+
+  const double res_M = dyadic_to_double(p.res_m, p.res_e), low_M = dyadic_to_double(p.low_m, p.low_e);
+  const int relu_floor = p.relu ? 0 : (int)0x80000000;
+  uint8_t* gy = reinterpret_cast<uint8_t*>(p.out) + (size_t)n0 * 2;
+
+  with_rq<true>(pol, p, [&](auto rq) {
+    int ymax = 0;
+    for (int j = 0; j < T; ++j) {
+      const int m0 = (rt0 + j * rstep) * BM;
+      if constexpr (DUAL) {
+#pragma unroll
+        for (int i = 0; i < NACC; ++i) acc[i] = 0;
+        for (int kt = 0; kt < KT2; ++kt) consume();
+#pragma unroll
+        for (int ni = 0; ni < NT; ++ni) {
+          const int col = ni * 8 + 2 * t;
+          const int4 r0 = *reinterpret_cast<const int4*>(&cs.rc[col]);
+          const int4 r1 = *reinterpret_cast<const int4*>(&cs.rc[col + 1]);
+          const double2 M1 = *reinterpret_cast<const double2*>(&cs.M1[col]);
+#pragma unroll
+          for (int hf = 0; hf < 2; ++hf) {
+            const int row = warp * 16 + hf * 8 + g;
+            const bool ok = m0 + row < p.M;
+            const int i0 = ni * 4 + hf * 2;
+            *reinterpret_cast<int2*>(smem + S::I_OFF + ((ni * 2 + hf) * CONV_THREADS + tid) * 8) =
+                make_int2(rq.term(rq.of_i32(sat_add(acc[i0], r0.x)), M1.x, r0.y, r0.z, ok),
+                          rq.term(rq.of_i32(sat_add(acc[i0 + 1], r1.x)), M1.y, r1.y, r1.z, ok));
+          }
+        }
+      }
+#pragma unroll
+      for (int i = 0; i < NACC; ++i) acc[i] = 0;
+      for (int kt = 0; kt < KT; ++kt) consume();
+
+      uint8_t* sY = smem + S::Y_OFF + (DUAL ? 0 : (j & 1) * S::Y_SLOT);
+#pragma unroll
+      for (int ni = 0; ni < NT; ++ni) {
+        const int col = ni * 8 + 2 * t;
+        const int4 c0 = *reinterpret_cast<const int4*>(&cs.chan[col]);
+        const int4 c1 = *reinterpret_cast<const int4*>(&cs.chan[col + 1]);
+        const double2 M = *reinterpret_cast<const double2*>(&cs.M[col]);
+        const double2 Cb = *reinterpret_cast<const double2*>(&cs.Cb[col]);
+#pragma unroll
+        for (int hf = 0; hf < 2; ++hf) {
+          const int row = warp * 16 + hf * 8 + g;
+          const bool ok = m0 + row < p.M;
+          const int i0 = ni * 4 + hf * 2;
+          uint32_t* yp = reinterpret_cast<uint32_t*>(sY + row * S::Y_PITCH + col * 2);
+          int32_t t0, t1;
+          if constexpr (DUAL) {
+            const int2 it = *reinterpret_cast<const int2*>(smem + S::I_OFF + ((ni * 2 + hf) * CONV_THREADS + tid) * 8);
+            t0 = it.x;
+            t1 = it.y;
+          } else {
+            const uint32_t pr = *yp;
+            t0 = rq.term(rq.of_u16(pr & 0xFFFFu), res_M, p.res_m, p.res_e, ok);
+            t1 = rq.term(rq.of_u16(pr >> 16), res_M, p.res_m, p.res_e, ok);
+          }
+          const int y0 = residual_y(rq, t0, acc[i0], Cb.x, c0, M.x, ok, relu_floor);
+          const int y1 = residual_y(rq, t1, acc[i0 + 1], Cb.y, c1, M.y, ok, relu_floor);
+          *yp = stream16_pair(y0, y1, ok, ymax);
+          if (p.low_bits != 0) stage_low_pair(sOut, S::OUT_PITCH, row, col, residual_low(rq, y0, low_M, p), residual_low(rq, y1, low_M, p));
+        }
+      }
+      __syncthreads();
+      copy_out_rows(sY, S::Y_PITCH, gy, (size_t)p.Cout * 2, BN * 2, m0, p.M);
+      if (p.low_bits != 0) copy_out_low<BN>(sOut, S::OUT_PITCH, reinterpret_cast<uint8_t*>(p.out_low), p.low_bits, m0, n0, p.M, p.Cout);
+    }
+    residual_flags(p, ymax, rq.ovf);
+  });
+  cp_async_wait<0>();
+}
+
+}
```

Result: faster. 29130, median of 6 (+15.2%).
